# HSarham/automatic-ar

Hardware: AMD Instinct MI355X
Metric: LM iterations/sec (higher is better)
Workload: dtype f64

## Files before the change

automatic-ar_amd/csrc/ba_capi.hip:

```cpp
#include <hip/hip_runtime.h>
#include <dlfcn.h>
#include <execinfo.h>
#include <fcntl.h>
#include <unistd.h>
#include <signal.h>

#include <algorithm>
#include <array>
#include <atomic>
#include <chrono>
#include <cmath>
#include <cstring>
#include <map>
#include <numeric>
#include <condition_variable>
#include <mutex>
#include <vector>

#include "../host/internal.h"
#include "../host/se3.h"
#include "geom.hpp"
#include "hostcopy.h"
#include "kernels.h"

// ... 910 lines not shown
    return AAR_OK;
}

void aar_lm_default_params(aar_lm_params *p) {
    p->max_iters = 10000;
    p->min_error = 1e-5;
    p->min_step_error_diff = 0;
    p->min_average_step_error_diff = 1e-4;
    p->tau = 1;
    p->verbose = 0;
}

void aar_problem_destroy(aar_problem *pb) {
    if (!pb) return;
    (void)hipSetDevice(pb->device);
    if (pb->stream) (void)hipStreamSynchronize(pb->stream);
    for (void *p : pb->allocs) (void)hipFree(p);
    if (pb->h_scal) (void)hipHostFree(pb->h_scal);
    if (pb->h_pcg) (void)hipHostFree(pb->h_pcg);
    if (pb->h_gather) (void)hipHostFree(pb->h_gather);
    if (pb->up_ev) (void)hipEventDestroy(pb->up_ev);
    if (pb->ev[0]) (void)hipEventDestroy(pb->ev[0]);
    if (pb->ev[1]) (void)hipEventDestroy(pb->ev[1]);
    for (hipEvent_t e : pb->ev_pool) (void)hipEventDestroy(e);
    if (pb->ev_fork) (void)hipEventDestroy(pb->ev_fork);
    if (pb->ev_join) (void)hipEventDestroy(pb->ev_join);
    if (pb->stream2) { (void)hipStreamSynchronize(pb->stream2); (void)hipStreamDestroy(pb->stream2); }
    if (pb->stream) (void)hipStreamDestroy(pb->stream);
    delete pb;
}

void aar_solver_default_options(aar_solver_options *o) {
    if (!o) return;
    memset(o, 0, sizeof *o);
    o->struct_size = (uint32_t)sizeof *o;
    o->solver = AAR_SOLVER_AUTO;
}

int aar_problem_create(const aar_problem_desc *d, aar_problem **out) { return aar_problem_create_ex(d, nullptr, out); }

static int problem_create(const aar_problem_desc *d, const aar_solver_options *opts, const aar_problem_constraints *cons, aar_problem **out);
namespace {
aar_problem_constraints constraints_of(const aar_problem_constraints *c) {
    aar_problem_constraints k;
    memset(&k, 0, sizeof k);
    if (c) memcpy(&k, c, std::min<size_t>(c->struct_size, sizeof k));
    k.struct_size = (uint32_t)sizeof k;
    return k;
}
bool constraints_empty(const aar_problem_constraints &k) { return k.n_fixed_cams == 0 && k.n_fixed_markers == 0 && k.n_priors == 0; }
bool info_psd(const double *I) {
    double scale = 0;
    for (int i = 0; i < 36; i++) scale = std::max(scale, std::fabs(I[i]));
    for (int i = 0; i < 6; i++)
        for (int j = 0; j < i; j++)
            if (std::fabs(I[6 * i + j] - I[6 * j + i]) > 1e-12 * scale) return false;
    if (scale == 0) return true;
    const double tol = 1e-13 * scale;
    double Lm[36] = {0}, D[6];
    for (int k = 0; k < 6; k++) {
        double d = I[6 * k + k];
        for (int j = 0; j < k; j++) d -= Lm[6 * k + j] * Lm[6 * k + j] * D[j];
        if (d < -tol) return false;
        for (int i = k + 1; i < 6; i++) {
            double v = I[6 * i + k];
            for (int j = 0; j < k; j++) v -= Lm[6 * i + j] * Lm[6 * k + j] * D[j];
            if (d <= tol) {
                if (std::fabs(v) > std::sqrt(tol * scale)) return false;
                Lm[6 * i + k] = 0;
            } else {
                Lm[6 * i + k] = v / d;
            }
        }
        D[k] = d <= tol ? 0.0 : d;
    }
    return true;
}
}

int aar_problem_constraints_validate(const aar_problem_desc *d, const aar_problem_constraints *cons) {
    if (!d) return set_error(AAR_ERR_INVALID, "aar_problem_constraints_validate: null problem description");
    if (!cons) return AAR_OK;
    if (cons->struct_size < sizeof(uint32_t) + sizeof(int32_t)) return set_error(AAR_ERR_INVALID, "aar_problem_constraints.struct_size is not set");
    const aar_problem_constraints k = constraints_of(cons);
    const int C = d->num_cams, M = d->num_markers;
    if (k.n_fixed_cams < 0 || k.n_fixed_markers < 0 || k.n_priors < 0) return set_error(AAR_ERR_INVALID, "aar_problem_constraints: negative count");
    if ((k.n_fixed_cams && !k.fixed_cams) || (k.n_fixed_markers && !k.fixed_markers) || (k.n_priors && !k.priors))
        return set_error(AAR_ERR_INVALID, "aar_problem_constraints: null array with a non-zero count");
    std::vector<uint8_t> fixed((size_t)std::max(C, 0) + std::max(M, 0), 0);
    for (int c = 0; c < C; c++) fixed[c] = (c == d->root_cam || !d->optimize_cam_poses) ? 1 : 0;
    for (int m = 0; m < M; m++) fixed[(size_t)C + m] = (m == d->root_marker || !d->optimize_marker_poses) ? 1 : 0;
    for (int i = 0; i < k.n_fixed_cams; i++) {
        const int c = k.fixed_cams[i];
        if (c < 0 || c >= C) return set_error(AAR_ERR_INVALID, "fixed_cams[%d] = %d: camera index out of range [0, %d)", i, c, C);
        fixed[c] = 1;
    }
    for (int i = 0; i < k.n_fixed_markers; i++) {
        const int m = k.fixed_markers[i];
        if (m < 0 || m >= M) return set_error(AAR_ERR_INVALID, "fixed_markers[%d] = %d: marker index out of range [0, %d)", i, m, M);
        fixed[(size_t)C + m] = 1;
    }
    std::vector<int32_t> owner(fixed.size(), -1);
    for (int p = 0; p < k.n_priors; p++) {
        const aar_pose_prior &q = k.priors[p];
        const char *what = q.kind == AAR_PRIOR_CAMERA ? "camera" : "marker";
        if (q.kind != AAR_PRIOR_CAMERA && q.kind != AAR_PRIOR_MARKER) return set_error(AAR_ERR_INVALID, "priors[%d]: kind %d is not AAR_PRIOR_CAMERA or AAR_PRIOR_MARKER", p, q.kind);
        const int lim = q.kind == AAR_PRIOR_CAMERA ? C : M;
        if (q.index < 0 || q.index >= lim) return set_error(AAR_ERR_INVALID, "priors[%d]: %s index %d out of range [0, %d)", p, what, q.index, lim);
        const size_t e = q.kind == AAR_PRIOR_CAMERA ? (size_t)q.index : (size_t)C + q.index;
        if (owner[e] >= 0) return set_error(AAR_ERR_INVALID, "priors[%d]: %s index %d already has a prior (priors[%d])", p, what, q.index, owner[e]);
        owner[e] = p;
        if (fixed[e]) return set_error(AAR_ERR_INVALID, "priors[%d]: %s index %d is fixed (root, non-optimised group or fixed index)", p, what, q.index);
        for (int i = 0; i < 6; i++)
            if (!std::isfinite(q.x6[i])) return set_error(AAR_ERR_INVALID, "priors[%d]: x6[%d] is not finite", p, i);
        for (int i = 0; i < 36; i++)
            if (!std::isfinite(q.info[i])) return set_error(AAR_ERR_INVALID, "priors[%d]: info[%d] is not finite", p, i);
        if (!info_psd(q.info)) return set_error(AAR_ERR_INVALID, "priors[%d]: the information matrix is not symmetric positive semi-definite (its Cholesky fails)", p);
    }
    return AAR_OK;
}

int aar_problem_create_constrained(const aar_problem_desc *d, const aar_solver_options *opts, const aar_problem_constraints *cons, aar_problem **out) {
    if (!d || !out) return set_error(AAR_ERR_INVALID, "aar_problem_create_constrained: null argument");
    int rc = aar_problem_constraints_validate(d, cons);
    if (rc) return rc;
    if (!cons || constraints_empty(constraints_of(cons))) return aar_problem_create_ex(d, opts, out);
    const aar_problem_constraints k = constraints_of(cons);
    return problem_create(d, opts, &k, out);
}

int32_t aar_problem_num_priors(const aar_problem *pb) { return pb ? pb->P.n_prior : 0; }

static int abort_bt_fd = 2;
static void abort_backtrace(int sig) {
    void *bt[64];
    { char msg[64]; const int k = aar::g_last_kernel_id; int n = 0; const char *t = "last kernel id "; while (t[n]) { msg[n] = t[n]; n++; } if (k < 0) msg[n++] = '-'; else { if (k >= 10) msg[n++] = '0' + k / 10; msg[n++] = '0' + k % 10; } msg[n++] = '\n'; (void)!write(abort_bt_fd, msg, n); }
    const int n = backtrace(bt, 64);
    backtrace_symbols_fd(bt, n, abort_bt_fd);
    signal(sig, SIG_DFL);
    raise(sig);
}

int aar_problem_create_ex(const aar_problem_desc *d, const aar_solver_options *opts, aar_problem **out) { return problem_create(d, opts, nullptr, out); }

static int problem_create(const aar_problem_desc *d, const aar_solver_options *opts, const aar_problem_constraints *cons, aar_problem **out) {
    { static bool once = false; if (!once && getenv("AAR_ABORT_BACKTRACE")) { once = true; const int fd = open(getenv("AAR_ABORT_BACKTRACE"), O_WRONLY | O_CREAT | O_APPEND, 0644); if (fd >= 0) abort_bt_fd = fd; signal(SIGABRT, abort_backtrace); } }
    if (!d || !out) return set_error(AAR_ERR_INVALID, "aar_problem_create: null argument");
    aar_solver_options so;
    aar_solver_default_options(&so);
    if (opts) {
        if (opts->struct_size < 2 * sizeof(uint32_t)) return set_error(AAR_ERR_INVALID, "aar_solver_options.struct_size is not set (use aar_solver_default_options)");
        memcpy(&so, opts, std::min<size_t>(opts->struct_size, sizeof so));
        so.struct_size = (uint32_t)sizeof so;
    }
    int env_over = 0;
    if (const char *e = getenv("AAR_SOLVER")) {
        if (so.solver == AAR_SOLVER_AUTO) {
            int v = -1;
            if (!strcmp(e, "direct")) v = AAR_SOLVER_DIRECT;
            else if (!strcmp(e, "pcg")) v = AAR_SOLVER_PCG;
            else if (!strcmp(e, "spcg")) v = AAR_SOLVER_SPCG;
            if (v >= 0) { so.solver = v; env_over |= AAR_ENV_SOLVER; }
        }
    }
    if (const char *e = getenv("AAR_DETERMINISTIC")) if (!so.deterministic && atoi(e) != 0) { so.deterministic = 1; env_over |= AAR_ENV_DETERMINISTIC; }
    if (const char *e = getenv("AAR_PCG_ETA")) if (so.pcg_eta == 0 && atof(e) > 0) { so.pcg_eta = atof(e); env_over |= AAR_ENV_PCG_ETA; }
    if (const char *e = getenv("AAR_PCG_MAX_IT")) if (so.pcg_max_it == 0 && atoi(e) > 0) { so.pcg_max_it = atoi(e); env_over |= AAR_ENV_PCG_MAX_IT; }
    if (so.solver < AAR_SOLVER_DIRECT || so.solver > AAR_SOLVER_AUTO) return set_error(AAR_ERR_INVALID, "aar_solver_options.solver %d is not one of AAR_SOLVER_*", so.solver);
    if (so.pcg_eta < 0 || so.pcg_max_it < 0 || so.pcg_eta_loose < 0 || so.pcg_eta_switch < 0 || so.pcg_abs_tol < 0) return set_error(AAR_ERR_INVALID, "aar_solver_options: negative pcg_eta / pcg_eta_loose / pcg_eta_switch / pcg_abs_tol / pcg_max_it");
    const int C = d->num_cams, M = d->num_markers, Fg = d->num_frames;
    const int64_t Ng = d->num_obs;
    if (C < 1 || M < 1 || Fg < 0 || Ng < 0) return set_error(AAR_ERR_INVALID, "aar_problem_create: bad sizes");
    if (d->root_cam < 0 || d->root_cam >= C || d->root_marker < 0 || d->root_marker >= M)
        return set_error(AAR_ERR_INVALID, "aar_problem_create: root index out of range");
    if (!d->cam_mats || (Ng > 0 && (!d->obs_frame || !d->obs_cam || !d->obs_marker || !d->obs_uv)))
        return set_error(AAR_ERR_INVALID, "aar_problem_create: null array");
    if (Ng >= (1LL << 31) || (int64_t)C + M >= 32768) return set_error(AAR_ERR_UNSUPPORTED, "problem too large for 32-bit indexing");
    std::vector<int64_t> per_frame(Fg, 0);
    int64_t global_slots = 0;
    {
        std::vector<int32_t> seen_c(C, -1), seen_m(M, -1);
        for (int64_t o = 0; o < Ng; o++) {
            const int f = d->obs_frame[o], c = d->obs_cam[o], m = d->obs_marker[o];
            if (f < 0 || f >= Fg || c < 0 || c >= C || m < 0 || m >= M) return set_error(AAR_ERR_INVALID, "observation %lld has an index out of range", (long long)o);
            if (o > 0 && f < d->obs_frame[o - 1]) return set_error(AAR_ERR_INVALID, "observations must be ordered by frame (reference residual order)");
            per_frame[f]++;
            if (seen_c[c] != f) { seen_c[c] = f; global_slots += d->optimize_cam_intrinsics ? 2 : 1; }
            if (seen_m[m] != f) { seen_m[m] = f; global_slots += 1; }
        }
    }
    int rc = ensure_device(d->device_id);
    if (rc) return rc;

    aar_problem *pb = new aar_problem();
    pb->device = d->device_id;
    pb->comm = d->comm;
    aar_lm_default_params(&pb->prm);
    memset(&pb->times, 0, sizeof pb->times);
    const char *tenv = getenv("AAR_STAGE_TIMERS");
    pb->stage_timers = tenv && tenv[0] == '1';
    auto fail = [&](int code) { aar_problem_destroy(pb); return code; };
    if (hipStreamCreateWithFlags(&pb->stream, hipStreamNonBlocking) != hipSuccess) return fail(set_error(AAR_ERR_HIP, "hipStreamCreate failed"));
    (void)hipEventCreate(&pb->ev[0]);
    (void)hipEventCreate(&pb->ev[1]);
    if (hipStreamCreateWithFlags(&pb->stream2, hipStreamNonBlocking) != hipSuccess ||
        hipEventCreateWithFlags(&pb->ev_fork, hipEventDisableTiming) != hipSuccess ||
        hipEventCreateWithFlags(&pb->ev_join, hipEventDisableTiming) != hipSuccess)
        return fail(set_error(AAR_ERR_HIP, "second stream / events could not be created"));
    { const char *e = getenv("AAR_OVERLAP"); pb->overlap = (e && e[0] == '1'); }
    { const char *e = getenv("AAR_MERGE_PASSES"); if (e) pb->merge_passes = (e[0] != '0'); }
    { const char *e = getenv("AAR_FUSED_COMM"); if (e) pb->fused_comm = (e[0] != '0'); }
    { const char *e = getenv("AAR_SPEC_CHOL"); if (e) pb->spec_chol = (e[0] != '0'); }

    PoseLayout &L = pb->L;
    L.C = C; L.M = M; L.F = Fg; L.rc = d->root_cam; L.rm = d->root_marker;
    L.oc = d->optimize_cam_poses != 0; L.om = d->optimize_marker_poses != 0; L.of = d->optimize_object_poses != 0;
    L.oi = d->optimize_cam_intrinsics != 0;
    pb->N_global = Ng;

    const int world = pb->comm ? pb->comm->world : 1, rank = pb->comm ? pb->comm->rank : 0;
    pb->P.pcg_rank0 = rank == 0 ? 1 : 0;
    std::vector<int32_t> begin(world + 1, 0);
    if ((rc = aar_plan_shards(Fg, per_frame.data(), world, begin.data()))) return fail(rc);
    pb->f_begin = begin[rank];
    pb->f_end = begin[rank + 1];
    int64_t ob = 0;
    for (int f = 0; f < pb->f_begin; f++) ob += per_frame[f];
    int64_t N = 0;
    for (int f = pb->f_begin; f < pb->f_end; f++) N += per_frame[f];
    pb->o_begin = ob;

    DeviceProblem &P = pb->P;
    P.intr = L.oi ? 1 : 0;
    P.C = C; P.M = M; P.A = C + M + (L.oi ? C : 0); P.F = pb->f_end - pb->f_begin; P.N = N;
    P.n = 6 * P.A;
    P.nT = (P.n + CHOL_NB - 1) / CHOL_NB;
    P.n_pad = P.nT * CHOL_NB;
    P.spcg_root_c = (L.oc && C > 1) ? L.rc : -1;
    P.spcg_root_m = (L.om && M > 1) ? C + L.rm : -1;
    P.spcg_n_free = (L.oc ? C - 1 : 0) + (L.om ? M - 1 : 0) + (L.oi ? C : 0);
    P.res_f32 = d->residual_mode == AAR_RES_F64 ? 0 : 1;
    pb->with_huber = d->with_huber != 0;
    P.huber = pb->with_huber ? pb->hubber_delta : -1.f;
    P.half_size = (double)((float)d->marker_size / 2.f);
    P.frames_fixed = L.of ? 0 : 1;
    const int A = P.A, F = P.F;
    std::vector<int32_t> held(C + M, 0);
    bool held_extra = false;
    if (cons) {
        for (int i = 0; i < cons->n_fixed_cams; i++) { const int c = cons->fixed_cams[i]; if (c != L.rc && L.oc) { held[c] = 1; held_extra = true; } }
        for (int i = 0; i < cons->n_fixed_markers; i++) { const int m = cons->fixed_markers[i]; if (m != L.rm && L.om) { held[C + m] = 1; held_extra = true; } }
    }

    int local_rc = AAR_OK;
    std::vector<int32_t> frame_obs_start(F + 1, 0), fslot_start(F + 1, 0), fslot_ent;
    std::vector<ObsIdx> a_idx(N);
    std::vector<float> a_uv((size_t)8 * N);
    if (N) memcpy(a_uv.data(), d->obs_uv + 8 * ob, sizeof(float) * 8 * N);
    {
        int64_t o = 0;
        std::vector<int32_t> slot_of(A, -1);
        for (int f = 0; f < F; f++) {
            frame_obs_start[f] = (int32_t)o;
            const int64_t cnt = per_frame[pb->f_begin + f];
            std::vector<int32_t> ents;
            for (int64_t k = 0; k < cnt; k++) {
                const int64_t g = ob + o + k;
                ents.push_back(d->obs_cam[g]);
                ents.push_back(C + d->obs_marker[g]);
                if (L.oi) ents.push_back(C + M + d->obs_cam[g]);
            }
            std::sort(ents.begin(), ents.end());
            ents.erase(std::unique(ents.begin(), ents.end()), ents.end());
            if (ents.size() >= (1u << SLOT_C_BITS) && !local_rc) local_rc = set_error(AAR_ERR_UNSUPPORTED, "frame %d touches %zu entities (limit %d)", f, ents.size(), (1 << SLOT_C_BITS) - 1);
            for (size_t s = 0; s < ents.size(); s++) slot_of[ents[s]] = (int32_t)s;
            for (int64_t k = 0; k < cnt; k++) {
                const int64_t g = ob + o + k;
                ObsIdx id;
                id.frame = f; id.cam = d->obs_cam[g]; id.marker = C + d->obs_marker[g];
                id.slots = pack_slots(slot_of[id.cam], slot_of[id.marker], L.oi ? slot_of[C + M + id.cam] : 0);
                a_idx[o + k] = id;
            }
            fslot_start[f] = (int32_t)fslot_ent.size();
            fslot_ent.insert(fslot_ent.end(), ents.begin(), ents.end());
            P.max_kf = std::max<int>(P.max_kf, (int)ents.size());
            o += cnt;
        }
        frame_obs_start[F] = (int32_t)o;
        fslot_start[F] = (int32_t)fslot_ent.size();
    }
    P.total_slots = (int)fslot_ent.size();
    std::vector<int32_t> frame_stride(F, 1);
    for (int f = 0; f < F; f++) {
        const int n = frame_obs_start[f + 1] - frame_obs_start[f];
        if (n <= 16) continue;
        int st = n / 8 + 1;
        while (std::gcd(st, n) != 1) st++;
        frame_stride[f] = st;
    }
    {
        auto env_int = [](const char *name, int &v) { if (const char *e = getenv(name)) v = atoi(e); };
        env_int("AAR_FUSED_PANEL", P.tune.fused_panel); env_int("AAR_BS_RIDES", P.tune.bs_rides); env_int("AAR_BACKSUB_RIDES", P.tune.backsub_rides);
        env_int("AAR_LDL_LOOKAHEAD", P.tune.lookahead); env_int("AAR_PASSA_VARIANT", P.tune.passA_variant); env_int("AAR_PACK_SYSTEM", P.tune.pack_system);
        env_int("AAR_INIT_HEADSTART", P.tune.init_headstart); env_int("AAR_PASSB_LEAN", P.tune.passB_lean); env_int("AAR_PASSA_WRENCH", P.tune.passA_wrench); env_int("AAR_PASSB_WRENCH_MERGED", P.tune.passB_wrench_merged); env_int("AAR_SPCG_BACKSUB_RIDES", P.tune.spcg_backsub_rides); env_int("AAR_PASSAB_OCC2", P.tune.passAB_occ2);
    }
    const size_t ldsA = P.tune.passA_wrench ? passA_wrench_lds_bytes(P.max_kf, L.oi)
                                            : std::max(passA_lds_bytes(P.max_kf, 256), passA_lds_bytes(P.max_kf, 64));
    if (ldsA > 160 * 1024 && !local_rc) local_rc = set_error(AAR_ERR_UNSUPPORTED, "a frame touches %d cameras+markers: %zu bytes of LDS in the frame-block kernel (%s form), the CU has 160 KiB", P.max_kf, ldsA, P.tune.passA_wrench ? "wrench" : "row");
    P.deterministic = so.deterministic ? 1 : 0;
    { const char *e = getenv("AAR_DENSE_FROM_PASSA"); if (e) P.dense_from_passA = atoi(e) != 0 ? 1 : 0; }
    {
        hipDeviceProp_t prop;
        const int cus = (hipGetDeviceProperties(&prop, pb->device) == hipSuccess && prop.multiProcessorCount > 0) ? prop.multiProcessorCount : 64;
        P.n_cus = cus;
        const bool pcg_ok = pcg_lds_bytes(A) <= 150 * 1024;
        if (const char *t = getenv("AAR_SPCG_COARSE")) P.spcg_coarse = atoi(t) != 0;
        if (const char *t = getenv("AAR_SPCG_COARSE_FROM")) P.spcg_coarse_from = atoi(t);
        if (const char *t = getenv("AAR_PCG_COARSE")) P.pcg_coarse = atoi(t) != 0;
        if (const char *t = getenv("AAR_PCG_COARSE_FROM")) P.pcg_coarse_from = atoi(t);
        if (held_extra) { P.spcg_coarse = 0; P.pcg_coarse = 0; }
        P.pcg_e_every = P.total_slots >= 300000 ? 3 : 1;
        if (const char *t = getenv("AAR_PCG_E_EVERY")) P.pcg_e_every = std::max(1, atoi(t));
        if (const char *t = getenv("AAR_PCG_RESIDENT")) P.pcg_resident = atoi(t) != 0;
        if (pcg_lds_bytes(A, true) > 150 * 1024) P.pcg_coarse = 0;
        const int spcg_per_cu = spcg_fits(P.nT) ? spcg_resident_per_cu(P.nT, spcg_coarse_now(P)) : 0;
        const bool spcg_ok = spcg_fits(P.nT) && P.n_pad / 6 <= std::max(1, spcg_per_cu) * cus;
        int solver = so.solver;
        if (solver == AAR_SOLVER_AUTO) {
            const double kf_avg = Fg > 0 ? (double)global_slots / (double)Fg : 0.0;
            const bool pcg_pays = A >= 96 && pcg_ok && (double)global_slots / (double)world * (kf_avg - 30.0) >= 4e6;
            if (P.nT < 2) solver = AAR_SOLVER_DIRECT;
            else if (spcg_ok && !pcg_pays) solver = AAR_SOLVER_SPCG;
            else if (pcg_ok) solver = AAR_SOLVER_PCG;
            else solver = AAR_SOLVER_DIRECT;
        }
        pb->solver = solver;
        pb->env_overrides = env_over;
        P.use_pcg = solver == AAR_SOLVER_PCG ? 1 : 0;
        P.use_spcg = solver == AAR_SOLVER_SPCG ? 1 : 0;
        if (const char *t = getenv("AAR_SPCG_SPREAD")) P.spcg_spread = std::max(1, atoi(t));
        if (P.n_pad / 6 > std::min(4, std::max(1, spcg_per_cu)) * (cus / 8)) P.spcg_spread = 1;
        P.pcg_eta = P.use_spcg ? SPCG_ETA_DEFAULT : PCG_ETA_DEFAULT;
        if (so.pcg_eta > 0) P.pcg_eta = so.pcg_eta;
        P.pcg_eta_loose = 0.0;
        if (so.pcg_eta_loose > 0) P.pcg_eta_loose = so.pcg_eta_loose;
        else if (so.pcg_eta == 0 && (P.use_pcg || P.use_spcg)) P.pcg_eta_loose = P.use_pcg ? PCG_ETA_LOOSE_DEFAULT : SPCG_ETA_LOOSE_DEFAULT;
        if (const char *e = getenv("AAR_PCG_ETA_LOOSE")) if (so.pcg_eta_loose == 0) P.pcg_eta_loose = atof(e);
        if (P.pcg_eta_loose <= P.pcg_eta) P.pcg_eta_loose = 0.0;
        P.pcg_abs_tol = P.use_pcg ? PCG_ABS_TOL_DEFAULT : SPCG_ABS_TOL_DEFAULT;
        if (so.pcg_abs_tol > 0) P.pcg_abs_tol = so.pcg_abs_tol;
        else if (const char *e = getenv("AAR_PCG_ABS_TOL")) P.pcg_abs_tol = atof(e);
        if (so.pcg_eta_switch > 0) P.pcg_eta_switch = so.pcg_eta_switch;
        else if (const char *e = getenv("AAR_PCG_ETA_SWITCH")) P.pcg_eta_switch = atof(e);
        P.pcg_eta_now = P.pcg_eta;
        P.spcg_max_it = spcg_default_cap(P.nT);
        if (so.pcg_max_it > 0) { P.pcg_max_it = so.pcg_max_it; P.spcg_max_it = std::min(so.pcg_max_it, SPCG_MAX_IT); }
        if (P.use_pcg && !pcg_ok && !local_rc) local_rc = set_error(AAR_ERR_UNSUPPORTED, "AAR_SOLVER_PCG keeps the CG vectors and the preconditioner of %d unknowns in LDS: too many shared entities", 6 * A);
        if (P.use_spcg && !spcg_ok && !local_rc) local_rc = set_error(AAR_ERR_UNSUPPORTED, "AAR_SOLVER_SPCG keeps the reduced system in the registers of one wavefront per shared entity: %d unknowns are too many (limit %d, and at most %d entities)", 6 * A, 96 * SPCG_MAX_NT, std::max(1, spcg_per_cu) * cus);
    }
    bool schur_mfma = A >= 96 && F > 0;
    if (const char *e = getenv("AAR_SCHUR_MFMA")) schur_mfma = atoi(e) != 0 && F > 0;
    if (P.deterministic) schur_mfma = false;
    if (P.use_pcg) schur_mfma = true;
    if (schur_mfma) {
        const size_t panel_bytes = (size_t)2 * F * ((A + 1 + 31) / 32 * 32) * 288;
        size_t free_b = 0, total_b = 0;
        size_t budget = (hipMemGetInfo(&free_b, &total_b) == hipSuccess) ? free_b / 2 : (size_t)64 << 30;
        if (const char *e = getenv("AAR_SCHUR_PANEL_MB")) budget = (size_t)std::max(0, atoi(e)) << 20;
        if (panel_bytes > budget) schur_mfma = false;
    }
    if (!schur_mfma && (size_t)A * 36 * 8 + 2048 > 160 * 1024 && !local_rc)
        local_rc = set_error(AAR_ERR_UNSUPPORTED, "%d cameras+markers exceed the row panel the output-stationary Schur kernel holds in LDS (and the dense panels of the MFMA kernel do not fit the memory budget)", A);
    {
        if (pb->comm && (rc = dev_alloc(pb, &pb->d_status, 1))) return fail(rc);
        int agreed = local_rc;
        if ((rc = collective_status(pb, local_rc, &agreed))) return fail(rc);
        if (local_rc) return fail(local_rc);
        if (agreed) return fail(set_error(agreed, "another rank could not create its shard of the problem (status %d)", agreed));
    }

    std::vector<int32_t> perm(N);
    std::iota(perm.begin(), perm.end(), 0);
    std::stable_sort(perm.begin(), perm.end(), [&](int32_t x, int32_t y) {
        const ObsIdx &p = a_idx[x], &q = a_idx[y];
        if (p.cam != q.cam) return p.cam < q.cam;
        if (p.marker != q.marker) return p.marker < q.marker;
        return p.frame < q.frame;
    });
    std::vector<ObsIdx> b_idx(N);
    std::vector<float> b_uv((size_t)8 * N);
    for (int64_t i = 0; i < N; i++) {
        b_idx[i] = a_idx[perm[i]];
        memcpy(&b_uv[8 * i], &a_uv[8 * (size_t)perm[i]], 8 * sizeof(float));
    }
    int chunk_len = (int)((N / 2048 + 63) / 64 * 64);
    chunk_len = std::min(std::max(chunk_len, 64), 512);
    if (const char *e = getenv("AAR_PASSB_CHUNK")) chunk_len = std::min(std::max(atoi(e) / 64 * 64, 64), PASSB_CHUNK);
    std::vector<int32_t> chunk_start;
    for (int64_t i = 0; i < N;) {
        int64_t e = i;
        while (e < N && b_idx[e].cam == b_idx[i].cam && b_idx[e].marker == b_idx[i].marker) e++;
        for (int64_t s = i; s < e; s += chunk_len) chunk_start.push_back((int32_t)s);
        i = e;
    }
    P.n_chunks = (int)chunk_start.size();
    chunk_start.push_back((int32_t)N);

    std::vector<int32_t> up_start(A + 1, 0), up_ent;
    {
        std::vector<std::vector<int32_t>> nb(A);
        for (int ch = 0; ch < P.n_chunks; ch++) {
            const ObsIdx &h = b_idx[chunk_start[ch]];
            if (ch > 0 && b_idx[chunk_start[ch - 1]].cam == h.cam && b_idx[chunk_start[ch - 1]].marker == h.marker) continue;
            int ents[3] = {h.cam, h.marker, L.oi ? C + M + h.cam : -1};
            for (int x = 0; x < 3; x++)
                for (int y = 0; y < 3; y++)
                    if (x != y && ents[x] >= 0 && ents[y] >= 0) nb[ents[x]].push_back(ents[y]);
        }
        for (int a = 0; a < A; a++) {
            std::sort(nb[a].begin(), nb[a].end());
            nb[a].erase(std::unique(nb[a].begin(), nb[a].end()), nb[a].end());
            up_start[a] = (int32_t)up_ent.size();
            up_ent.insert(up_ent.end(), nb[a].begin(), nb[a].end());
        }
        up_start[A] = (int32_t)up_ent.size();
        if (up_ent.empty()) up_ent.push_back(0);
    }

    std::vector<std::vector<std::pair<int32_t, int32_t>>> inc(A);
    for (int f = 0; f < F; f++)
        for (int s = fslot_start[f]; s < fslot_start[f + 1]; s++) inc[fslot_ent[s]].push_back({f, s});
    std::vector<int4> pair_rec;
    std::vector<int32_t> sw_ent, sw_begin, sw_end;
    const int64_t total_pairs = P.total_slots;
    int per_item = (int)std::min<int64_t>(64, std::max<int64_t>(16, total_pairs / 1024));
    per_item = (per_item + 3) / 4 * 4;
    if (const char *e = getenv("AAR_SCHUR_ITEM")) per_item = std::max(4, atoi(e));
    std::vector<int> pair_base(A + 1, 0);
    for (int a = 0; a < A; a++) {
        pair_base[a] = (int)pair_rec.size();
        for (auto &pr : inc[a]) pair_rec.push_back(make_int4(pr.first, pr.second, fslot_start[pr.first], 0));
    }
    pair_base[A] = (int)pair_rec.size();
    int window = 0;
    if (total_pairs >= 262144) window = 64;
    if (const char *e = getenv("AAR_SCHUR_WINDOW")) window = std::max(0, atoi(e));
    if (window > 0) {
        std::vector<int> cursor(A, 0);
        for (int f0 = 0; f0 < F; f0 += window)
            for (int a = 0; a < A; a++) {
                int c = cursor[a];
                const int cnt = (int)inc[a].size();
                int e = c;
                while (e < cnt && inc[a][e].first < f0 + window) e++;
                if (e > c) {
                    sw_ent.push_back(a);
                    sw_begin.push_back(pair_base[a] + c);
                    sw_end.push_back(pair_base[a] + e);
                }
                cursor[a] = e;
            }
    } else {
        int xcd = 1;
        if (const char *e = getenv("AAR_SCHUR_XCD")) xcd = atoi(e) != 0 ? 8 : 1;
        std::vector<std::vector<std::array<int32_t, 3>>> lists(xcd);
        for (int a = 0; a < A; a++) {
            const int cnt = (int)inc[a].size();
            int s = 0;
            for (int x = 0; x < xcd; x++) {
                const int f_hi = (int)((int64_t)F * (x + 1) / xcd);
                int e = s;
                while (e < cnt && inc[a][e].first < f_hi) e++;
                for (int c = s; c < e; c += per_item)
                    lists[x].push_back({(int32_t)a, (int32_t)(pair_base[a] + c), (int32_t)(pair_base[a] + std::min(e, c + per_item))});
                s = e;
            }
        }
        size_t longest = 0;
        for (auto &l : lists) longest = std::max(longest, l.size());
        for (size_t k = 0; k < longest; k++)
            for (int x = 0; x < xcd; x++) {
                if (k < lists[x].size()) { sw_ent.push_back(lists[x][k][0]); sw_begin.push_back(lists[x][k][1]); sw_end.push_back(lists[x][k][2]); }
                else if (xcd > 1) { sw_ent.push_back(0); sw_begin.push_back(0); sw_end.push_back(0); }
            }
    }
    P.n_swork = (int)sw_ent.size();
    std::vector<int64_t> sp_off;
    std::vector<int32_t> se_start, se_items, pbr_start, pbr_chunk, pbr_kind, pbr_a, pbr_b;
    int64_t sp_total = 0;
    if (P.deterministic) {
        sp_off.resize(sw_ent.size());
        std::vector<std::vector<int32_t>> items(A);
        for (size_t w = 0; w < sw_ent.size(); w++) {
            sp_off[w] = sp_total;
            sp_total += ((int64_t)(sw_ent[w] + 1) * 36 + 8);
            items[sw_ent[w]].push_back((int32_t)w);
        }
        se_start.assign(A + 1, 0);
        for (int a = 0; a < A; a++) {
            std::sort(items[a].begin(), items[a].end(), [&](int32_t x, int32_t y) { return sw_begin[x] < sw_begin[y]; });
            se_start[a] = (int32_t)se_items.size();
            se_items.insert(se_items.end(), items[a].begin(), items[a].end());
        }
        se_start[A] = (int32_t)se_items.size();
        std::vector<std::vector<int32_t>> by_cam(C), by_mk(A);
        pbr_start.push_back(0);
        auto emit = [&](int kind, int ea, int eb, const std::vector<int32_t> &chs) {
            if (chs.empty()) return;
            pbr_chunk.insert(pbr_chunk.end(), chs.begin(), chs.end());
            pbr_start.push_back((int32_t)pbr_chunk.size());
            pbr_kind.push_back(kind); pbr_a.push_back(ea); pbr_b.push_back(eb);
        };
        std::vector<int32_t> run;
        for (int ch = 0; ch < P.n_chunks; ch++) {
            const ObsIdx &h = b_idx[chunk_start[ch]];
            by_cam[h.cam].push_back(ch);
            by_mk[h.marker].push_back(ch);
            run.push_back(ch);
            const bool last = ch + 1 == P.n_chunks || b_idx[chunk_start[ch + 1]].cam != h.cam || b_idx[chunk_start[ch + 1]].marker != h.marker;
            if (last) { emit(2, h.cam, h.marker, run); run.clear(); }
        }
        for (int c = 0; c < C; c++) emit(0, c, 0, by_cam[c]);
        for (int m = 0; m < A; m++) emit(1, m, 0, by_mk[m]);
        P.n_pbr = (int)pbr_kind.size();
        P.pb_stride = L.oi ? 152 : 90;
    }
    std::vector<int32_t> sm_ga, sm_gb, sm_fb, sm_fe, slot_frame, slot_dense, dense_ent;
    std::vector<int32_t> sm_frames;
    if (schur_mfma && !P.use_pcg) {
        std::vector<int32_t> seen;
        for (int a = 0; a < A; a++)
            if (!inc[a].empty()) seen.push_back(a);
        std::stable_sort(seen.begin(), seen.end(), [&](int32_t x, int32_t y) { return inc[x].size() > inc[y].size(); });
        std::vector<int32_t> dense_of(A, -1);
        dense_ent.push_back(-1);
        for (int32_t a : seen) { dense_of[a] = (int32_t)dense_ent.size(); dense_ent.push_back(a); }
        P.Ad = ((int)dense_ent.size() + 31) / 32 * 32;
        dense_ent.resize(P.Ad, -1);
        const int nga = P.Ad / 16, ngb = P.Ad / 32;
        std::vector<std::vector<uint8_t>> pa(nga, std::vector<uint8_t>(F, 0)), pb(ngb, std::vector<uint8_t>(F, 0));
        for (int f = 0; f < F; f++) {
            pa[0][f] = pb[0][f] = 1;
            for (int s = fslot_start[f]; s < fslot_start[f + 1]; s++) {
                const int dd = dense_of[fslot_ent[s]];
                pa[dd / 16][f] = 1;
                pb[dd / 32][f] = 1;
            }
        }
        struct Blk { int ga, gb; std::vector<int32_t> fr; };
        std::vector<Blk> blks;
        int64_t total_steps = 0;
        for (int ga = 0; ga < nga; ga++)
            for (int gb = 0; gb <= (16 * ga + 15) / 32; gb++) {
                Blk bk{ga, gb, {}};
                for (int f = 0; f < F; f++)
                    if (pa[ga][f] && pb[gb][f]) bk.fr.push_back(f);
                if (bk.fr.empty()) continue;
                total_steps += ((int64_t)bk.fr.size() + 1) / 2;
                blks.push_back(std::move(bk));
            }
        int target = 12 * (int)blks.size();
        if (const char *e = getenv("AAR_SCHUR_SPLIT")) target = std::max(1, atoi(e)) * (int)blks.size();
        const int64_t plen = std::max<int64_t>(16, ((2 * total_steps + target - 1) / target + 3) / 4 * 4);
        struct Piece { int blk; int64_t b, e; int f0; };
        std::vector<Piece> pieces;
        for (size_t k = 0; k < blks.size(); k++)
            for (int64_t b0 = 0; b0 < (int64_t)blks[k].fr.size(); b0 += plen)
                pieces.push_back({(int)k, b0, std::min<int64_t>(b0 + plen, (int64_t)blks[k].fr.size()), blks[k].fr[b0]});
        std::stable_sort(pieces.begin(), pieces.end(), [](const Piece &x, const Piece &y) { return x.f0 < y.f0; });
        for (const Piece &pc : pieces) {
            sm_ga.push_back(blks[pc.blk].ga); sm_gb.push_back(blks[pc.blk].gb);
            sm_fb.push_back((int32_t)sm_frames.size());
            sm_frames.insert(sm_frames.end(), blks[pc.blk].fr.begin() + pc.b, blks[pc.blk].fr.begin() + pc.e);
            sm_fe.push_back((int32_t)sm_frames.size());
        }
        slot_frame.resize(P.total_slots);
        slot_dense.resize(P.total_slots);
        for (int f = 0; f < F; f++)
            for (int s = fslot_start[f]; s < fslot_start[f + 1]; s++) {
                slot_frame[s] = f;
                slot_dense[s] = dense_of[fslot_ent[s]];
            }
        P.n_smwork = (int)sm_ga.size();
    }

    std::vector<int32_t> ent_fixed(A, 0);
    for (int c = 0; c < C; c++) ent_fixed[c] = (c == L.rc || !L.oc) ? 1 : 0;
    for (int m = 0; m < M; m++) ent_fixed[C + m] = (m == L.rm || !L.om) ? 1 : 0;
    for (int e = 0; e < C + M; e++) ent_fixed[e] |= held[e];
    std::vector<double> Kh(d->cam_mats, d->cam_mats + 9 * (size_t)C);

#define UP(field, vec) if ((rc = dev_upload(pb, &P.field, vec))) return fail(rc)
    UP(K, Kh); UP(a_idx, a_idx); UP(a_uv, a_uv); UP(frame_obs_start, frame_obs_start); UP(frame_stride, frame_stride);
    UP(fslot_start, fslot_start); UP(fslot_ent, fslot_ent); UP(b_idx, b_idx); UP(b_uv, b_uv);
    UP(chunk_start, chunk_start); UP(ent_fixed, ent_fixed); UP(up_start, up_start); UP(up_ent, up_ent);
    UP(sw_ent, sw_ent); UP(sw_begin, sw_begin); UP(sw_end, sw_end); UP(pair_rec, pair_rec);
    if (P.use_pcg) {
        const int cus = P.n_cus;
        int64_t longest = 0;
        for (int a = 0; a < A; a++) longest = std::max<int64_t>(longest, pair_base[a + 1] - pair_base[a]);
        int64_t chunk = std::max<int64_t>(256, (total_pairs + 2LL * cus - 1) / (2LL * cus));
        chunk = std::max<int64_t>(chunk, (longest + 7) / 8);
        if (const char *t = getenv("AAR_PCG_CHUNK")) chunk = std::max<int64_t>((longest + 7) / 8, atoll(t));
        std::vector<int32_t> it_ent, it_begin, it_end, ent_item_start(A + 1, 0);
        for (int a = 0; a < A; a++) {
            ent_item_start[a] = (int32_t)it_ent.size();
            const int64_t b0 = pair_base[a], e0 = ent_fixed[a] ? pair_base[a] : pair_base[a + 1];
            int64_t b = b0;
            do {
                const int64_t e = std::min<int64_t>(e0, b + chunk);
                it_ent.push_back(a); it_begin.push_back((int32_t)b); it_end.push_back((int32_t)e);
                b = e;
            } while (b < e0);
        }
        ent_item_start[A] = (int32_t)it_ent.size();
        P.pcg_n_items = (int)it_ent.size();
        UP(pcg_it_ent, it_ent); UP(pcg_it_begin, it_begin); UP(pcg_it_end, it_end); UP(pcg_ent_item_start, ent_item_start);
    }
    if (P.deterministic) { UP(sp_off, sp_off); UP(se_start, se_start); UP(se_items, se_items); UP(pbr_start, pbr_start); UP(pbr_chunk, pbr_chunk); UP(pbr_kind, pbr_kind); UP(pbr_a, pbr_a); UP(pbr_b, pbr_b); }
    if (P.n_smwork) { UP(sm_ga, sm_ga); UP(sm_gb, sm_gb); UP(sm_fb, sm_fb); UP(sm_fe, sm_fe); UP(slot_dense, slot_dense); UP(slot_frame, slot_frame); UP(dense_ent, dense_ent); UP(sm_frames, sm_frames); }
#undef UP
#define AL(field, count) if ((rc = dev_alloc(pb, &P.field, (size_t)(count)))) return fail(rc)
    AL(z[0], 6 * (size_t)(A + F)); AL(z[1], 6 * (size_t)(A + F));
    AL(ent[0], (size_t)(A + F) * ENT_STRIDE); AL(ent[1], (size_t)(A + F) * ENT_STRIDE);
    for (int w = 0; w < 2; w++) {
        AL(blk[w].V, (size_t)F * 36); AL(blk[w].gf, (size_t)F * 6); AL(blk[w].W, (size_t)P.total_slots * 36);
        AL(blk[w].Vinv, (size_t)F * 36); AL(blk[w].hf, (size_t)F * 6);
        AL(blk[w].S, (size_t)P.n_pad * P.n_pad + 2 * (size_t)P.n_pad + 8);
        P.blk[w].rhs = P.blk[w].S + (size_t)P.n_pad * P.n_pad;
        P.blk[w].g0 = P.blk[w].rhs + P.n_pad;
        P.blk[w].tail = P.blk[w].g0 + P.n_pad;
        if (hipMemset(P.blk[w].tail, 0, 8 * sizeof(double)) != hipSuccess) return fail(set_error(AAR_ERR_HIP, "hipMemset failed"));
    }
    if (P.deterministic) { AL(sp_part, (size_t)sp_total); AL(pb_part, (size_t)P.n_chunks * P.pb_stride); }
    if (P.use_pcg) {
        AL(pcg_ws, (size_t)P.pcg_n_items * 28 + 6 * (size_t)F + 8); AL(pcg_counter, 8);
        AL(pcg_yg, (size_t)3 * PCG_NYV * P.n_pad + (size_t)28 * A + 160 + 8); AL(pcg_hop, 2 * PCG_HOP_WORDS);
        if (const char *t = getenv("AAR_PCG_FUSED")) P.pcg_fused = atoi(t) != 0 ? 1 : 0;
        {
            int w32 = 1;
            if (const char *t = getenv("AAR_PCG_W32")) w32 = atoi(t) != 0 ? 1 : 0;
            if (w32 && P.pcg_fused && !P.deterministic && P.pcg_eta >= PCG_W32_MIN_ETA)
                for (int w = 0; w < 2; w++) AL(blk[w].Wf, (size_t)P.total_slots * 36 + 4);
        }
        P.pcg_grid = P.n_cus;
        const int64_t want = std::max<int64_t>(32, ((int64_t)F + 3) / 4);
        P.pcg_grid = (int)std::min<int64_t>(P.pcg_grid, want);
        if (pb->comm) {
            AL(pcgd_setup, (size_t)A * 28 + 152); AL(pcgd_minv, (size_t)A * 36 + 72 + (size_t)12 * A + 8);
            AL(pcgd_state, 2 * (18 * (size_t)A + 8)); AL(pcgd_y, 3 * (6 * (size_t)A + 8));
            if (hipHostMalloc((void **)&pb->h_pcg, 8 * sizeof(double), hipHostMallocMapped | hipHostMallocCoherent) != hipSuccess)
                return fail(set_error(AAR_ERR_HIP, "hipHostMalloc failed"));
            memset(pb->h_pcg, 0, 8 * sizeof(double));
            if (hipHostGetDevicePointer((void **)&P.pcgd_host, pb->h_pcg, 0) != hipSuccess) return fail(set_error(AAR_ERR_HIP, "hipHostGetDevicePointer failed"));
        }
        if (const char *t = getenv("AAR_PCG_GRID")) P.pcg_grid = std::max(1, atoi(t));
        P.pcg_grid = std::min(P.pcg_grid, pcg_max_grid(A, P.pcg_coarse != 0, P.n_cus));
    }
    if (P.use_spcg) {
        AL(spcg_ws, spcg_ws_doubles(P.n_pad)); AL(spcg_iters, 8); AL(spcg_done, 2);
        if (spcg_coarse_now(P)) AL(spcg_pre, spcg_pre_doubles(P.n_pad));
        spcg_ws_reset(P, pb->stream);
    }
    if (P.n_smwork) { AL(Wd, (size_t)F * P.Ad * 36); AL(Yd, (size_t)F * P.Ad * 36); }
    AL(Dfac, (size_t)P.nT * CHOL_NB * CHOL_NB); AL(Linv16, (size_t)P.nT * (CHOL_NB / 16) * 256); AL(delta_s, P.n_pad); AL(bs_flags, (size_t)P.nT + 1);
    AL(Lp, (size_t)P.nT * P.n_pad * CHOL_NB); AL(zf, P.n_pad);
    AL(err_part, std::max<size_t>((size_t)F, (size_t)((N + 255) / 256)) + 1);
    AL(lin_part, 2 * (size_t)(F + 1)); AL(scal, 8); AL(flags, 4);
    if (cons && cons->n_priors > 0) {
        const int np_ = cons->n_priors;
        std::vector<int32_t> pent(np_);
        std::vector<double> pdat((size_t)np_ * PRIOR_DAT);
        for (int p = 0; p < np_; p++) {
            const aar_pose_prior &q = cons->priors[p];
            pent[p] = q.kind == AAR_PRIOR_CAMERA ? q.index : C + q.index;
            memcpy(&pdat[(size_t)p * PRIOR_DAT], q.x6, 6 * sizeof(double));
            memcpy(&pdat[(size_t)p * PRIOR_DAT + 6], q.info, 36 * sizeof(double));
        }
        if ((rc = dev_upload(pb, &P.prior_ent, pent)) || (rc = dev_upload(pb, &P.prior_dat, pdat))) return fail(rc);
        AL(prior_out, (size_t)np_ * 8 + 1);
        P.n_prior = np_;
        P.prior_rank0 = rank == 0 ? 1 : 0;
        pb->priors.assign(cons->priors, cons->priors + np_);
    }
#undef AL
    if ((rc = dev_alloc(pb, &pb->d_diag, P.n_pad))) return fail(rc);
    if (pb->comm && (rc = dev_alloc(pb, &pb->d_frames_all, 6 * (size_t)std::max(Fg, 1)))) return fail(rc);
    if (pb->comm && (rc = dev_alloc(pb, &pb->d_pack, (size_t)P.n_pad * (P.n_pad + 1) / 2 + 2 * (size_t)P.n_pad + 8))) return fail(rc);
    if (hipHostMalloc((void **)&pb->h_scal, 16 * sizeof(double), hipHostMallocMapped | hipHostMallocCoherent) != hipSuccess)
        return fail(set_error(AAR_ERR_HIP, "hipHostMalloc failed"));
    memset(pb->h_scal, 0, 16 * sizeof(double));
    if (hipHostGetDevicePointer((void **)&P.host_result, pb->h_scal, 0) != hipSuccess)
        return fail(set_error(AAR_ERR_HIP, "hipHostGetDevicePointer failed"));
    if (hipStreamSynchronize(pb->stream) != hipSuccess) return fail(set_error(AAR_ERR_HIP, "upload failed"));
    {
        if (pb->h_z.reserve((size_t)6 * (A + F))) return fail(set_error(AAR_ERR_HIP, "hipHostMalloc(pose staging) failed"));
        if (hipEventCreateWithFlags(&pb->up_ev, hipEventDisableTiming) != hipSuccess) { pb->up_ev = nullptr; (void)hipGetLastError(); }
        if (hipMemcpyAsync(pb->h_z.data(), P.z[0], (size_t)6 * (A + F) * sizeof(double), hipMemcpyDeviceToHost, pb->stream) != hipSuccess ||
            hipStreamSynchronize(pb->stream) != hipSuccess)
            return fail(set_error(AAR_ERR_HIP, "device-to-host copy failed"));
    }
    pb->h_fslot_start = fslot_start;
    pb->h_fslot_ent = fslot_ent;
    pb->h_ent_fixed = ent_fixed;
    *out = pb;
    return AAR_OK;
}

int64_t aar_problem_full_len(const aar_problem *pb) { return pb->L.full_len(); }
int64_t aar_problem_num_vars(const aar_problem *pb) { return pb->L.z_len(); }
int64_t aar_problem_local_obs(const aar_problem *pb) { return pb->P.N; }

int aar_problem_set_huber_delta(aar_problem *pb, float delta) {
    if (!pb || !(delta > 0.f)) return set_error(AAR_ERR_INVALID, "aar_problem_set_huber_delta: bad argument");
    pb->hubber_delta = delta;
    if (pb->with_huber) pb->P.huber = delta;
    return AAR_OK;
}
float aar_problem_get_huber_delta(const aar_problem *pb) { return pb ? pb->hubber_delta : 0.f; }

int aar_eval_residuals(aar_problem *pb, const double *x_full, double *r, double *sum_sq) {
    if (!pb || !x_full) return set_error(AAR_ERR_INVALID, "aar_eval_residuals: null argument");
    if (r && pb->comm) return set_error(AAR_ERR_UNSUPPORTED, "residual vector output is single-GPU only");
    HIP_TRY(hipSetDevice(pb->device));
    DeviceProblem &P = pb->P;
    int rc = upload_z(pb, x_full, pb->cur);
    if (rc) return rc;
    double *d_r = nullptr;
    if (r) HIP_TRY(hipMalloc((void **)&d_r, std::max<size_t>(1, 8 * (size_t)P.N) * sizeof(double)));
    launch_unpack(P, pb->cur, pb->stream);
    launch_residual(P, pb->cur, d_r, pb->stream);
    HIP_TRY(hipMemsetAsync(P.lin_part, 0, 2 * (size_t)(P.F + 1) * sizeof(double), pb->stream));
    launch_reduce_scalars(P, residual_blocks(P), false, 0ull, pb->stream);
    rc = allreduce(pb, P.scal, 1, NCCL_SUM);
    if (rc) { if (d_r) (void)hipFree(d_r); return rc; }
    pb->seq++;
    launch_publish(P, pb->seq, pb->stream);
    HIP_TRY(hipStreamSynchronize(pb->stream));
    if (r && (rc = copy_d2h(pb, r, d_r, 8 * (size_t)P.N * sizeof(double)))) { (void)hipFree(d_r); return rc; }
    if ((rc = wait_result(pb))) { if (d_r) (void)hipFree(d_r); return rc; }
    if (d_r) (void)hipFree(d_r);
    if (sum_sq) *sum_sq = pb->h_scal[0];
    pb->lm_ready = false;
    return check_async("residual kernels");
}

int aar_reproj_stats(aar_problem *pb, const double *x_full, double *rmse, double *sum_sq) {
    if (!pb) return set_error(AAR_ERR_INVALID, "aar_reproj_stats: null argument");
    const int saved = pb->P.res_f32;
    const float saved_h = pb->P.huber;
    pb->P.res_f32 = 0;
    pb->P.huber = -1.f;
    double ss = 0;
    int rc = aar_eval_residuals(pb, x_full, nullptr, &ss);
    pb->P.res_f32 = saved;
    pb->P.huber = saved_h;
    if (rc) return rc;
    if (sum_sq) *sum_sq = ss;
    if (rmse) *rmse = std::sqrt(ss / (4.0 * (double)pb->N_global));
    return AAR_OK;
}

int aar_eval_normal_equations(aar_problem *pb, const double *x_full, double *JtJ, double *B, double *sum_sq) {
    if (!pb || !x_full) return set_error(AAR_ERR_INVALID, "aar_eval_normal_equations: null argument");
    if (pb->comm) return set_error(AAR_ERR_UNSUPPORTED, "dense normal-equation output is single-GPU only");
    HIP_TRY(hipSetDevice(pb->device));
    DeviceProblem &P = pb->P;
    const PoseLayout &L = pb->L;
    int rc = upload_z(pb, x_full, pb->cur);
    if (rc) return rc;
    if ((rc = zero_block_set(pb, pb->cur))) return rc;
    P.want_w64 = 1;
    rc = eval_blocks(pb, pb->cur, -1.0, -1);
    P.want_w64 = 0;
    if (rc) return rc;
    const int A = P.A, F = P.F, np = P.n_pad;
    const DeviceProblem::Blocks &bk = P.blk[pb->cur];
    std::vector<double> U0((size_t)np * np), g0(np), V((size_t)F * 36), gf((size_t)F * 6), W((size_t)P.total_slots * 36), ep(n_err_terms(P));
    HIP_TRY(hipStreamSynchronize(pb->stream));
    if ((rc = copy_d2h(pb, U0.data(), bk.S, U0.size() * sizeof(double))) || (rc = copy_d2h(pb, g0.data(), bk.g0, g0.size() * sizeof(double)))) return rc;
    if (F) {
        if ((rc = copy_d2h(pb, V.data(), bk.V, V.size() * sizeof(double))) || (rc = copy_d2h(pb, gf.data(), bk.gf, gf.size() * sizeof(double))) ||
            (rc = copy_d2h(pb, W.data(), bk.W, W.size() * sizeof(double)))) return rc;
    }
    if (!ep.empty() && (rc = copy_d2h(pb, ep.data(), P.err_part, ep.size() * sizeof(double)))) return rc;
    pb->lm_ready = false;
    const int64_t Pz = L.z_len();
    auto par_col = [&](int a, int i) -> int64_t {
        if (a < L.C) { const int s = L.cam_slot(a); return (s < 0 || !L.oc) ? -1 : L.z_cam0() + 6LL * s + i; }
        if (a < L.C + L.M) { const int s = L.mk_slot(a - L.C); return (s < 0 || !L.om) ? -1 : L.z_mk0() + 6LL * s + i; }
        return i < 4 ? L.z_intr0() + 9LL * (a - L.C - L.M) + i : -1;
    };
    if (JtJ) {
        std::fill(JtJ, JtJ + Pz * Pz, 0.0);
        for (int a = 0; a < A; a++)
            for (int b = 0; b <= a; b++)
                for (int i = 0; i < 6; i++)
                    for (int j = 0; j < 6; j++) {
                        if (a == b && j > i) continue;
                        const int64_t ca = par_col(a, i), cb = par_col(b, j);
                        if (ca < 0 || cb < 0) continue;
                        const double v = U0[(size_t)(6 * a + i) * np + 6 * b + j];
                        JtJ[ca * Pz + cb] = v;
                        JtJ[cb * Pz + ca] = v;
                    }
        if (L.of)
            for (int f = 0; f < F; f++) {
                const int64_t cf = L.z_fr0() + 6LL * f;
                for (int i = 0; i < 6; i++)
                    for (int j = 0; j < 6; j++) JtJ[(cf + i) * Pz + cf + j] = V[(size_t)f * 36 + i * 6 + j];
                for (int s = pb->h_fslot_start[f]; s < pb->h_fslot_start[f + 1]; s++)
                    for (int i = 0; i < 6; i++) {
                        const int64_t ca = par_col(pb->h_fslot_ent[s], i);
                        if (ca < 0) continue;
                        for (int j = 0; j < 6; j++) {
                            const double v = W[(size_t)s * 36 + i * 6 + j];
                            JtJ[ca * Pz + cf + j] = v;
                            JtJ[(cf + j) * Pz + ca] = v;
                        }
                    }
            }
    }
    if (B) {
        std::fill(B, B + Pz, 0.0);
        for (int a = 0; a < A; a++)
            for (int i = 0; i < 6; i++) {
                const int64_t ca = par_col(a, i);
                if (ca >= 0) B[ca] = g0[6 * (size_t)a + i];
            }
        if (L.of)
            for (int f = 0; f < F; f++)
                for (int i = 0; i < 6; i++) B[L.z_fr0() + 6LL * f + i] = gf[(size_t)f * 6 + i];
    }
    if (sum_sq) {
        double s = 0;
        for (double v : ep) s += v;
        *sum_sq = s;
    }
    return AAR_OK;
}

int aar_problem_eval_priors(aar_problem *pb, const double *x_full, double *e_out, double *cost) {
    if (!pb || !x_full) return set_error(AAR_ERR_INVALID, "aar_problem_eval_priors: null argument");
    HIP_TRY(hipSetDevice(pb->device));
    DeviceProblem &P = pb->P;
    if (P.n_prior == 0) {
        if (cost) *cost = 0.0;
        return AAR_OK;
    }
    int rc = upload_z(pb, x_full, pb->cur);
    if (rc) return rc;
    pb->lm_ready = false;
    pb->blocks_valid = false;
    launch_unpack(P, pb->cur, pb->stream);
    launch_prior(P, pb->cur, false, pb->stream);
    pb->launches += 2;
    if ((rc = check_async("prior kernels"))) return rc;
    HIP_TRY(hipStreamSynchronize(pb->stream));
    std::vector<double> h((size_t)P.n_prior * 8 + 1);
    if ((rc = copy_d2h(pb, h.data(), P.prior_out, h.size() * sizeof(double)))) return rc;
    if (e_out)
        for (int p = 0; p < P.n_prior; p++) memcpy(e_out + 6 * (size_t)p, &h[8 * (size_t)p], 6 * sizeof(double));
    if (cost) *cost = h[(size_t)P.n_prior * 8];
    return AAR_OK;
}

int aar_eval_damped_step(aar_problem *pb, const double *x_full, double mu, double *delta) {
    if (!pb || !x_full || !delta) return set_error(AAR_ERR_INVALID, "aar_eval_damped_step: null argument");
    HIP_TRY(hipSetDevice(pb->device));
    const PoseLayout &L = pb->L;
    int rc = upload_z(pb, x_full, pb->cur);
    if (rc) return rc;
    if ((rc = zero_block_set(pb, pb->cur))) return rc;
    if ((rc = eval_blocks(pb, pb->cur, -1.0, -1))) return rc;
    pb->vinv_mu = -1;
    pb->schur_mu = -1;
    pb->s_reduced = pb->trial_reduced = false;
    pb->spcg_skip = pb->spcg_backoff = 0;
    pb->last_cg_its = -1;
    pb->near_cap_tries = 0;
    pb->P.spcg_coarse_on = 0;
    pb->P.pcg_e_age = 0;
    if (pb->P.use_pcg && pb->P.pcg_counter) HIP_TRY(hipMemsetAsync(pb->P.pcg_counter + 2, 0, sizeof(int32_t), pb->stream));
    pb->P.pcg_eta_now = pb->P.pcg_eta;
    if ((rc = damped_try_fb(pb, mu, false))) return rc == TRY_NOT_POSITIVE_DEFINITE ? AAR_ERR_NUMERIC : rc;
    pb->lm_ready = false;
    std::vector<double> x0(x_full, x_full + L.full_len()), x1(x0);
    if ((rc = download_z(pb, 1 - pb->cur, x1.data()))) return rc;
    std::vector<double> z0((size_t)std::max<int64_t>(L.z_len(), 1)), z1(z0);
    extract_z(L, x0.data(), z0.data());
    extract_z(L, x1.data(), z1.data());
    for (int64_t i = 0; i < L.z_len(); i++) delta[i] = z1[i] - z0[i];
    return AAR_OK;
}

int aar_problem_covariance(aar_problem *pb, const double *x_full, double *entity_cov, double *entity_diag, double *frame_cov,
                           aar_covariance_report *report) {
    if (!pb || !x_full) return set_error(AAR_ERR_INVALID, "aar_problem_covariance: null argument");
    if (report && report->struct_size < sizeof(uint32_t)) return set_error(AAR_ERR_INVALID, "aar_problem_covariance: report->struct_size not set");
    HIP_TRY(hipSetDevice(pb->device));
    DeviceProblem &P = pb->P;
    const PoseLayout &L = pb->L;
    const int cur = pb->cur, np = P.n_pad, n2 = P.n_pad + CHOL_NB, nT2 = P.nT + 1, NB = CHOL_NB;
    int rc = upload_z(pb, x_full, cur);
    if (rc) return rc;
    if ((rc = zero_block_set(pb, cur))) return rc;
    pb->lm_ready = false;
    pb->blocks_valid = false;
    pb->vinv_mu = pb->schur_mu = -1;
    pb->s_reduced = pb->trial_reduced = false;
    pb->spec_chol_blk = -1;
    if (pb->panels_blk == cur) pb->panels_blk = -1;
    P.want_w64 = 1;
    rc = eval_blocks(pb, cur, -1.0, -1);
    P.want_w64 = 0;
    if (rc) return rc;
    launch_frame_inv(P, cur, 0.0, pb->stream);
    launch_schur(P, cur, 1.0, pb->stream, 0, 0, nullptr, false);
    launch_reduce_scalars(P, n_err_terms(P), false, 0ull, pb->stream, P.blk[cur].tail);
    pb->launches += 3;
    if (pb->comm && (rc = allreduce_system(pb, cur, 1))) return rc;
    const size_t fr = (size_t)std::max(P.F, 1) * 36;
    const size_t o_S2 = 0, o_D = o_S2 + (size_t)n2 * n2 + 2 * (size_t)n2 + 8, o_Li = o_D + (size_t)nT2 * NB * NB, o_Lp = o_Li + (size_t)nT2 * (NB / 16) * 256,
                 o_zf = o_Lp + (size_t)nT2 * n2 * NB, o_ds = o_zf + n2, o_Lc = o_ds + n2, o_X = o_Lc + (size_t)np * np, o_Si = o_X + (size_t)np * np,
                 o_Dv = o_Si + (size_t)np * np, o_fr = o_Dv + np, o_db = o_fr + fr, total = o_db + 36 * (size_t)std::max(P.A, 1);
    if (!pb->cov_ws) {
        if ((rc = dev_alloc(pb, &pb->cov_ws, total))) return rc;
        if ((rc = dev_alloc(pb, &pb->cov_iws, (size_t)np + nT2 + 1 + 4))) return rc;
    }
    double *ws = pb->cov_ws;
    int32_t *rowmask = pb->cov_iws, *bsf = rowmask + np, *flg = bsf + nT2 + 1;
    HIP_TRY(hipMemcpy2DAsync(pb->d_diag, sizeof(double), P.blk[cur].S, (size_t)(np + 1) * sizeof(double), sizeof(double), np, hipMemcpyDeviceToDevice, pb->stream));
    std::vector<double> diag(np);
    double sum_sq = 0;
    HIP_TRY(hipStreamSynchronize(pb->stream));
    if ((rc = copy_d2h(pb, diag.data(), pb->d_diag, np * sizeof(double))) || (rc = copy_d2h(pb, &sum_sq, P.blk[cur].tail, sizeof(double)))) return rc;
    auto par_col = [&](int a, int i) -> int64_t {
        if (a < L.C) { const int s = L.cam_slot(a); return (s < 0 || !L.oc) ? -1 : L.z_cam0() + 6LL * s + i; }
        if (a < L.C + L.M) { const int s = L.mk_slot(a - L.C); return (s < 0 || !L.om) ? -1 : L.z_mk0() + 6LL * s + i; }
        return i < 4 ? L.z_intr0() + 9LL * (a - L.C - L.M) + i : -1;
    };
    std::vector<int32_t> mask(np, 1);
    for (int a = 0; a < P.A; a++) {
        bool seen = false;
        for (int i = 0; i < 6; i++) seen |= par_col(a, i) >= 0 && diag[6 * a + i] != 0.0;
        const bool held = a < L.C + L.M && pb->h_ent_fixed[a];
        for (int i = 0; i < 6; i++) mask[6 * a + i] = (seen && !held && par_col(a, i) >= 0) ? 0 : 1;
    }
    if ((rc = copy_h2d(pb, rowmask, mask.data(), np * sizeof(int32_t)))) return rc;
    double *S2 = ws + o_S2;
    launch_cov_stage(P.blk[cur].S, np, S2, n2, rowmask, pb->stream);
    HIP_TRY(hipMemsetAsync(S2 + (size_t)n2 * n2, 0, (2 * (size_t)n2 + 8) * sizeof(double), pb->stream));
    HIP_TRY(hipMemsetAsync(bsf, 0, (nT2 + 1 + 4) * sizeof(int32_t), pb->stream));
    DeviceProblem Q = P;
    Q.n_pad = n2; Q.nT = nT2;
    Q.blk[cur].S = S2; Q.blk[cur].rhs = S2 + (size_t)n2 * n2; Q.blk[cur].g0 = Q.blk[cur].rhs + n2; Q.blk[cur].tail = Q.blk[cur].g0 + n2;
    Q.Dfac = ws + o_D; Q.Linv16 = ws + o_Li; Q.Lp = ws + o_Lp; Q.zf = ws + o_zf; Q.delta_s = ws + o_ds; Q.bs_flags = bsf; Q.bs_epoch = 0; Q.flags = flg;
    (void)launch_chol(Q, cur, 0.0, pb->stream, -1);
    launch_cov_inverse(S2, Q.Dfac, Q.Lp, np, n2, nT2, P.tune.fused_panel, ws + o_Lc, ws + o_Dv, ws + o_X, ws + o_Si, pb->stream);
    const bool frames = frame_cov && L.of && P.F > 0;
    if (frames) launch_cov_frames(P, cur, ws + o_Si, rowmask, ws + o_fr, pb->stream);
    if (entity_diag && !entity_cov) launch_cov_diag_blocks(ws + o_Si, np, P.A, ws + o_db, pb->stream);
    pb->launches += 4 + 3 * nT2 + np / 32;
    if ((rc = check_async("covariance kernels"))) return rc;
// ... 1274 lines not shown
```

automatic-ar_amd/csrc/kernels.h:

```cpp
#pragma once
#include <hip/hip_runtime.h>
#include <stdint.h>
#include <utility>

namespace aar {

constexpr int CHOL_NB = 96;
constexpr int PASSB_CHUNK = 1024;
constexpr int SPCG_MAX_IT = 128, SPCG_BUFS = SPCG_MAX_IT + 2, SPCG_MAX_NT = 14;
inline int spcg_default_cap(int nT) { return nT <= 4 ? 64 : SPCG_MAX_IT; }
constexpr int PCG_NY = 16;
constexpr int PCG_NYV = 2;
constexpr int PCG_HOP_WORDS = (2 * PCG_NY + 1) * 16;
constexpr double PCG_W32_MIN_ETA = 1e-4;
constexpr double SPCG_ABS_TOL_DEFAULT = 2e-5, PCG_ABS_TOL_DEFAULT = 5e-5;
constexpr double SPCG_ETA_DEFAULT = 3e-4, SPCG_ETA_LOOSE_DEFAULT = 0.0, PCG_ETA_DEFAULT = 5e-3, PCG_ETA_LOOSE_DEFAULT = 0.0;
inline int spcg_stride(int n_pad) { return 8 * (n_pad / 6); }


#ifndef SPCG_PRE
#define SPCG_PRE 0
#endif

enum KernelId { KID_UNPACK = 0, KID_RESIDUAL, KID_PASSA, KID_PASSB, KID_MAXDIAG, KID_FRAME_INV, KID_SCHUR, KID_LDL_DIAG,
                KID_LDL_TRSM, KID_LDL_UPDATE, KID_LDL_BACKSOLVE, KID_BACKSUB, KID_REDUCE, KID_LDL_PANEL, KID_PCG, KID_SPCG, KID_SPCG_PRE, KID_PRIOR, KID_COUNT };

struct LaunchHook {
    void (*pre)(void *ctx, int kid) = nullptr;
    void (*post)(void *ctx, int kid) = nullptr;
    void *ctx = nullptr;
};

struct ObsIdx {
    int32_t frame, cam, marker, slots;
};

struct DeviceProblem {
    int C = 0, M = 0, A = 0;
    int intr = 0;
    int F = 0;
    int64_t N = 0;
    int n = 0, n_pad = 0, nT = 0;
    int total_slots = 0, max_kf = 0;
    int n_chunks = 0, n_swork = 0;
    int res_f32 = 1;
    float huber = -1.f;
    double half_size = 0;
    double *K = nullptr;
    ObsIdx *a_idx = nullptr;
    float *a_uv = nullptr;
    int32_t *frame_obs_start = nullptr;
    int32_t *frame_stride = nullptr;
    int32_t *fslot_start = nullptr;
    int32_t *fslot_ent = nullptr;
    ObsIdx *b_idx = nullptr;
    float *b_uv = nullptr;
    int32_t *chunk_start = nullptr;
    int32_t *ent_fixed = nullptr;
    int frames_fixed = 0;
    int32_t *sw_ent = nullptr, *sw_begin = nullptr, *sw_end = nullptr;
    int4 *pair_rec = nullptr;
    int n_smwork = 0;
    int32_t *sm_ga = nullptr, *sm_gb = nullptr, *sm_fb = nullptr, *sm_fe = nullptr, *sm_frames = nullptr;
    int Ad = 0;
    int32_t *slot_dense = nullptr;
    int32_t *slot_frame = nullptr;
    int32_t *dense_ent = nullptr;
    double *Wd = nullptr, *Yd = nullptr;
    int dense_from_passA = 1;
    int deterministic = 0;
    double *pb_part = nullptr;
    int pb_stride = 0, n_pbr = 0;
    int32_t *pbr_start = nullptr, *pbr_chunk = nullptr, *pbr_kind = nullptr, *pbr_a = nullptr, *pbr_b = nullptr;
    double *sp_part = nullptr;
    int64_t *sp_off = nullptr;
    int32_t *se_start = nullptr, *se_items = nullptr;
    int use_pcg = 0, pcg_grid = 0, pcg_max_it = 200;
    double pcg_eta = 0.1;
    double pcg_eta_loose = 0.0, pcg_eta_switch = 0.01, pcg_eta_now = 0.1;
    double pcg_abs_tol = SPCG_ABS_TOL_DEFAULT;
    int pcg_n_items = 0;
    int32_t *pcg_it_ent = nullptr, *pcg_it_begin = nullptr, *pcg_it_end = nullptr, *pcg_ent_item_start = nullptr;
    double *pcg_ws = nullptr;
    int32_t *pcg_counter = nullptr;
    mutable int pcg_parity = 0;
    int n_cus = 256;
    mutable int want_w64 = 0;
    int pcg_fused = 1;
    int pcg_rank0 = 1;
    int pcg_resident = 1;
    int pcg_e_every = 1;
    mutable int pcg_e_age = 0;
    int pcg_coarse = 1, pcg_coarse_from = 8;
    int32_t *up_start = nullptr, *up_ent = nullptr;
    double *pcg_yg = nullptr;
    int32_t *pcg_hop = nullptr;
    int use_spcg = 0, spcg_max_it = 64;
    int spcg_spread = 8;
    int spcg_coarse = 1;
    int spcg_coarse_from = 12;
    mutable int spcg_coarse_on = 0;
    double *spcg_pre = nullptr;
    mutable int spcg_pre_epoch = 0;
    int spcg_root_c = -1, spcg_root_m = -1, spcg_n_free = 0;
    int spcg_test_drop = -1;
    double *spcg_ws = nullptr;
    int32_t *spcg_iters = nullptr;
    mutable int spcg_parity = 0;
    int32_t *spcg_done = nullptr;
    mutable int spcg_epoch = 0;
    double *pcgd_setup = nullptr, *pcgd_minv = nullptr, *pcgd_state = nullptr, *pcgd_y = nullptr, *pcgd_host = nullptr;
    struct Tuning {
        int fused_panel = 3;
        int bs_rides = 1;
        int backsub_rides = 0;
        int lookahead = 1;
        int passA_variant = 0;
        int passAB_occ2 = -1;
        int spcg_backsub_rides = 0;
        int passA_wrench = 1;
        int passB_wrench_merged = 0;
        int passB_lean = 0;
        int pack_system = -1;
        int init_headstart = 1;
    } tune;
    double *z[2] = {nullptr, nullptr};
    double *ent[2] = {nullptr, nullptr};
    struct Blocks {
        double *V = nullptr, *gf = nullptr;
        double *W = nullptr;
        float *Wf = nullptr;
        double *Vinv = nullptr, *hf = nullptr;
        double *S = nullptr;
        double *rhs = nullptr;
        double *g0 = nullptr;
        double *tail = nullptr;
    } blk[2];
    double *Dfac = nullptr;
    double *Linv16 = nullptr;
    double *Lp = nullptr;
    double *zf = nullptr;
    double *delta_s = nullptr;
    int32_t *bs_flags = nullptr;
    mutable int bs_epoch = 0;
    double *err_part = nullptr;
    double *lin_part = nullptr;
    double *scal = nullptr;
    double *host_result = nullptr;
    int32_t *flags = nullptr;
    double *r_out = nullptr;
    int n_prior = 0, prior_rank0 = 1;
    int32_t *prior_ent = nullptr;
    double *prior_dat = nullptr;
    double *prior_out = nullptr;
    LaunchHook hook;
};

void raise_dynamic_lds(const void *kernel, size_t bytes);
template <typename... Params, typename... Args>
inline void launch_lds(void (*kernel)(Params...), dim3 grid, dim3 block, size_t lds, hipStream_t st, Args &&...args) {
    raise_dynamic_lds(reinterpret_cast<const void *>(kernel), lds);
    hipLaunchKernelGGL(kernel, grid, block, lds, st, std::forward<Args>(args)...);
}

struct KTable { const double *base; int stride; };
constexpr int ENT_STRIDE_H = 24;
inline KTable k_table(const DeviceProblem &P, int which) {
    if (P.intr) return KTable{P.ent[which] + (size_t)(P.C + P.M) * ENT_STRIDE_H, ENT_STRIDE_H};
    return KTable{P.K, 9};
}
constexpr int SLOT_C_BITS = 10, SLOT_M_BITS = 11;
inline int pack_slots(int sc, int sm, int sk) { return sc | (sm << SLOT_C_BITS) | (sk << (SLOT_C_BITS + SLOT_M_BITS)); }

extern volatile int g_last_kernel_id;
struct HookScope {
    const DeviceProblem &P;
    int kid;
    HookScope(const DeviceProblem &p, int k) : P(p), kid(k) { g_last_kernel_id = k; if (P.hook.pre) P.hook.pre(P.hook.ctx, kid); }
    ~HookScope() { if (P.hook.post) P.hook.post(P.hook.ctx, kid); }
};

void launch_unpack(const DeviceProblem &P, int which, hipStream_t st, int zero_blk = -1);
void launch_residual(const DeviceProblem &P, int which, double *r_out, hipStream_t st);
void launch_passA(const DeviceProblem &P, int which, double mu_pred, int zero_blk, hipStream_t st);
void launch_passB(const DeviceProblem &P, int which, hipStream_t st);
bool launch_passAB(const DeviceProblem &P, int which, double mu_pred, int zero_blk, hipStream_t st);
size_t passA_lds_bytes(int max_kf, int block);
size_t passA_wrench_lds_bytes(int max_kf, bool intr);
void launch_maxdiag(const DeviceProblem &P, int which, hipStream_t st);
void launch_frame_inv(const DeviceProblem &P, int which, double mu, hipStream_t st, const double *mu_dev = nullptr, double mu_scale = 0.0);
bool launch_schur(const DeviceProblem &P, int which, double sign, hipStream_t st, unsigned long long ride_seq = 0, int ride_n_err = 0,
                  double *ride_scal = nullptr, bool panels_ready = false);
bool launch_chol(const DeviceProblem &P, int which, double mu, hipStream_t st, int trial = -1);
void launch_backsub(const DeviceProblem &P, int cur, int trial, hipStream_t st);
void launch_pcg(const DeviceProblem &P, int which, double mu, hipStream_t st);
size_t pcg_lds_bytes(int A, bool coarse = false);
int pcg_max_grid(int A, bool coarse, int cus);
bool launch_spcg(const DeviceProblem &P, int which, double mu, hipStream_t st, int trial = -1);
int spcg_resident_per_cu(int nT, bool coarse);
inline bool spcg_coarse_now(const DeviceProblem &P) { return P.spcg_coarse && (P.spcg_root_c >= 0 || P.spcg_root_m >= 0); }
bool spcg_fits(int nT);
size_t spcg_ws_doubles(int n_pad);
size_t spcg_pre_doubles(int n_pad);
void spcg_ws_reset(const DeviceProblem &P, hipStream_t st);
void launch_pcgd_setup(const DeviceProblem &P, int which, double mu, hipStream_t st);
void launch_pcgd_iter(const DeviceProblem &P, int which, double mu, int k, bool last, unsigned long long publish_seq, hipStream_t st);
double *pcgd_y_of_launch(const DeviceProblem &P, int k);
void launch_reduce_scalars(const DeviceProblem &P, int n_err, bool fold_shared, unsigned long long publish_seq, hipStream_t st,
                           double *scal_out = nullptr, int maxdiag_blk = -1);
void launch_publish(const DeviceProblem &P, unsigned long long publish_seq, hipStream_t st, const double *src = nullptr, bool flags_reduced = false);
int residual_blocks(const DeviceProblem &P);
constexpr int PRIOR_DAT = 42;
void launch_prior(const DeviceProblem &P, int which, bool add, hipStream_t st);
inline int n_err_terms(const DeviceProblem &P) { return P.F + ((P.n_prior > 0 && P.prior_rank0) ? 1 : 0); }
void launch_track(const DeviceProblem &P, int which, int max_iters, double min_error, double min_step, double min_avg, double tau,
                  int32_t *iters_out, double *err_out, hipStream_t st);

constexpr int SMOOTH_TAIL = 256;
struct SmoothWork {
    double *z[2] = {nullptr, nullptr};
    double *delta = nullptr;
    double *Dg = nullptr, *Of = nullptr;
    double *rhs = nullptr;
    double *Dw = nullptr, *Uw = nullptr, *bw = nullptr, *Dinv = nullptr, *Ls = nullptr;
    double *Ef[2] = {nullptr, nullptr}, *Pe[2] = {nullptr, nullptr};
    double *lin = nullptr;
    double *lam = nullptr;
    double *rel_buf = nullptr;
    const double *rel = nullptr;
    double *res = nullptr;
    int32_t *flag = nullptr;
};
size_t smooth_work_doubles(int F);
void smooth_work_carve(SmoothWork &w, double *base, int F);
void launch_smooth_eval(const DeviceProblem &P, int which, const SmoothWork &w, int cur, bool with_j, hipStream_t st);
int launch_smooth_solve(const SmoothWork &w, int F, double mu, hipStream_t st);

constexpr int LIVE_MAX_W = 16;
constexpr int LIVE_HDR_BYTES = 64;
constexpr int LIVE_REC_BYTES = 48;
constexpr int LIVE_RES_DOUBLES = 24;
constexpr int LIVE_INFO_DOUBLES = 16;
inline size_t live_slot_bytes(int max_obs) {
    return (LIVE_HDR_BYTES + (size_t)(LIVE_REC_BYTES + sizeof(int32_t)) * (size_t)max_obs + 15) / 16 * 16;
}
struct LiveArgs {
    const double *ent, *Kmat;
    const char *ring;
    size_t slot_bytes;
    double *zslot;
    double *anchor;
    double *Ef, *Pe;
    double *res;
    float huber; double h;
    int max_iters; double min_error, min_step_error_diff, min_average_step_error_diff, tau;
    int W, slots, first_slot;
    int has_anchor, smooth, has_init;
    double rows;
    int cnt[LIVE_MAX_W];
    double lam[LIVE_MAX_W][2];
    int anchor_pair;
    int marginal, has_marginal;
    int covariance;
    double *unc;
};
constexpr int LIVE_UNC_VALID = 0, LIVE_UNC_HAS = 1, LIVE_UNC_DROP = 2, LIVE_UNC_LM = 4, LIVE_UNC_M = 40, LIVE_UNC_HDR = 48;
constexpr int LIVE_UNC_DOUBLES = LIVE_UNC_HDR + 36 * LIVE_MAX_W;
constexpr double LIVE_MARGINAL_PIVOT_REL = 1e-10;
void launch_live_push(const LiveArgs &a, hipStream_t st);

constexpr int LIVE_START_VOTE = 1, LIVE_START_BEST = 2;
struct LiveInitArgs {
    char *slot;
    int n_det;
    const void *cams;
    const double *Tcr, *Tmr;
    int C;
    float hf; double h;
    double threshold;
    int do_vote, policy, has_init, has_prev;
    const double *zprev;
    const double *ent, *Kmat; float huber; double h_track;
    double *poses; int *has2;
    double *Tc, *BJ, *cost; int *fin;
    double *info;
};
void launch_live_init(const LiveInitArgs &a, hipStream_t st);

void launch_cov_stage(const double *S, int n_pad, double *S2, int n2, const int32_t *rowmask, hipStream_t st);
void launch_cov_inverse(const double *S2, const double *Dfac, const double *Lp, int n_pad, int n2, int nT2, int fused_m, double *Lc, double *Dinv,
                        double *X, double *Sinv, hipStream_t st);
void launch_cov_diag_blocks(const double *Sinv, int n_pad, int A, double *out, hipStream_t st);
void launch_cov_frames(const DeviceProblem &P, int which, const double *Sinv, const int32_t *rowmask, double *out, hipStream_t st);

constexpr int RR_DIGIT_BITS = 11, RR_BINS = 1 << RR_DIGIT_BITS, RR_PASSES = 6;
struct RRSel {
    unsigned long long prefix, rank;
    double t;
    int pshift, done, single, pad;
};
struct RRWork {
    double *err = nullptr, *ss = nullptr, *fstat = nullptr, *rstat = nullptr, *esum = nullptr, *emax = nullptr, *hd = nullptr;
    uint8_t *keep = nullptr;
    int32_t *perm = nullptr, *run_start = nullptr, *cam_run_start = nullptr, *mk_run_start = nullptr, *mk_runs = nullptr;
    unsigned long long *rmax = nullptr;
    uint32_t *hist = nullptr;
    RRSel *sel = nullptr;
    int R = 0;
};
constexpr int RR_HIST_WORDS = RR_BINS + 3;
void launch_rr_errors(const DeviceProblem &P, int which, const RRWork &w, unsigned long long rank, hipStream_t st);
void launch_rr_select_pass(const DeviceProblem &P, const RRWork &w, hipStream_t st);
void launch_rr_to_double(const RRWork &w, hipStream_t st);
void launch_rr_pick(const RRWork &w, bool reduced, hipStream_t st);
void launch_rr_stats(const DeviceProblem &P, const RRWork &w, int has_rule, double k_median, double min_px, hipStream_t st);

__device__ __forceinline__ double encode_flags(int f) {
    return (double)(f & 1) + 4096.0 * (double)((f >> 1) & 1) + 16777216.0 * (double)((f >> 2) & 1) + 68719476736.0 * (double)((f >> 3) & 1);
}
__device__ __forceinline__ int decode_flags(double v) {
    const long long q = (long long)v;
    return ((q % 4096) ? 1 : 0) | (((q / 4096) % 4096) ? 2 : 0) | (((q / 16777216) % 4096) ? 4 : 0) | ((q / 68719476736LL) ? 8 : 0);
}

__device__ __forceinline__ void publish_host(const double *__restrict__ scal, const int32_t *__restrict__ flags,
                                             double *__restrict__ host, unsigned long long seq, int flags_reduced = 0) {
#pragma unroll
    for (int i = 0; i < 8; i++) host[i] = scal[i];
    reinterpret_cast<long long *>(host)[8] = flags_reduced ? (long long)decode_flags(scal[3]) : (long long)(flags[0] | flags[1] | flags[2] | flags[3]);
    __threadfence_system();
    __hip_atomic_store(reinterpret_cast<unsigned long long *>(host) + 9, seq, __ATOMIC_RELEASE, __HIP_MEMORY_SCOPE_SYSTEM);
}


}
```

automatic-ar_amd/csrc/spcg_kernels.hip:

```cpp
#include "geom.hpp"
#include "kernels.h"
#include "backsub.hpp"
#include "wave.hpp"

namespace aar {

namespace {

constexpr unsigned long long SPCG_EMPTY = 0xFFF85EEDFFF85EEDull;

__device__ __forceinline__ bool sp_empty(double v) { return (unsigned long long)__double_as_longlong(v) == SPCG_EMPTY; }
__device__ __forceinline__ void sp_st(double *p, double v) { __hip_atomic_store(p, v, __ATOMIC_RELAXED, __HIP_MEMORY_SCOPE_AGENT); }
__device__ __forceinline__ void sp_st_xcd(double *p, double v) { __hip_atomic_store(p, v, __ATOMIC_RELAXED, __HIP_MEMORY_SCOPE_WORKGROUP); }
__device__ __forceinline__ double sp_ld(const double *p) { return __hip_atomic_load(p, __ATOMIC_RELAXED, __HIP_MEMORY_SCOPE_AGENT); }

__device__ __forceinline__ double rl(double v, int l) {
    return __hiloint2double(__builtin_amdgcn_readlane(__double2hiint(v), l), __builtin_amdgcn_readlane(__double2loint(v), l));
}

}

#ifdef AAR_STAMPS
__device__ unsigned long long g_sp_stamps[512];
__device__ int g_sp_polls[80];
#define SP_STAMP(k) do { __builtin_amdgcn_sched_barrier(0); if (e == e0 && lane == 0 && (k) < 512) g_sp_stamps[k] = __builtin_amdgcn_s_memtime(); __builtin_amdgcn_sched_barrier(0); } while (0)
#define SP_VAL(k, v) do { if (e == e0 && lane == 0 && (k) < 512) g_sp_stamps[k] = (unsigned long long)__double_as_longlong(v); } while (0)
#else
#define SP_STAMP(k) do { } while (0)
#define SP_VAL(k, v) do { } while (0)
#endif

struct SpcgArgs {
    const double *S, *rhs, *g0;
    const int32_t *ent_fixed;
    int n, n_pad;
    double mu, eta2;
    double abs2_mu;
    int max_it;
    double *ws;
    long long set_len;
    int stride, parity;
    double *x_out;
    int32_t *iters;
    int32_t *flags;
    int spread;
    int ride, n_ent_total, n_riders;
    BacksubArgs bs;
    int32_t *done;
    int done_epoch;
    int test_drop;
    const double *pre_rows, *pre_minv, *pre_z, *pre_azt, *pre_share;
    int root_c, root_m;
    int C, M;
};

typedef unsigned int sp_u32x4 __attribute__((ext_vector_type(4)));

template <int NT, bool CO>
__global__ void __launch_bounds__(64) k_spcg(const SpcgArgs a) {
    constexpr int NPAD = 96 * NT, NK = 6 * NT, NENT = 16 * NT, NL = NT, NEB = (NENT + 63) / 64;
    __shared__ __align__(16) double mv[NPAD];
    if (blockIdx.x % a.spread || (int)blockIdx.x >= a.n_ent_total * a.spread) {
        if (!a.ride || blockIdx.x % 8 == 0) return;
        __shared__ double red[32];
        const int bx = (int)blockIdx.x, cg_range = a.n_ent_total * a.spread;
        const int rid = bx < cg_range ? bx - bx / a.spread - 1 : a.n_ent_total * (a.spread - 1) + (bx - cg_range) - (bx - cg_range + 7) / 8;
        for (int blk = rid; blk <= a.bs.n_frame_blocks; blk += a.n_riders) backsub_body(a.bs, blk, red, a.done + 1, a.done_epoch, a.flags);
        return;
    }
    const int lane = threadIdx.x, e = blockIdx.x / a.spread, i = lane >> 3, g = lane & 7;
    auto leave = [&]() {
        if (!a.ride) return;
        asm volatile("s_waitcnt vmcnt(0)" ::: "memory");
        if (lane == 0) {
            const int old = __hip_atomic_fetch_add(a.done, 1, __ATOMIC_RELAXED, __HIP_MEMORY_SCOPE_AGENT);
            if (old + 1 == a.done_epoch * a.n_ent_total) __hip_atomic_store(a.done + 1, a.done_epoch, __ATOMIC_RELAXED, __HIP_MEMORY_SCOPE_AGENT);
        }
    };
    const int n_free_ent = a.n / 6;
    auto fixed = [&](int ent) -> bool { return ent >= n_free_ent || (a.ent_fixed[ent < n_free_ent ? ent : 0] != 0 && !(CO && (ent == a.root_c || ent == a.root_m))); };
    double *set = a.ws + (size_t)a.parity * a.set_len, *other = a.ws + (size_t)(1 - a.parity) * a.set_len;
    const int nprev_raw = a.iters[0];
    {
        const int nprev = min(nprev_raw + 2, SPCG_BUFS);
        for (int bq = lane >> 3; bq < nprev; bq += 8) sp_st(other + (size_t)bq * a.stride + 8 * e + (lane & 7), __longlong_as_double((long long)SPCG_EMPTY));
    }
    if (fixed(e)) {
        if (lane < 6) sp_st(a.x_out + 6 * e + lane, 0.0);
        leave();
        return;
    }
    if (e == a.test_drop) return;
    int e0 = -1, n_act = 0;
#pragma unroll
    for (int k = 0; k < NEB; k++) {
        const unsigned long long fr = __ballot(lane + 64 * k < NENT && !fixed(lane + 64 * k));
        if (e0 < 0 && fr) e0 = 64 * k + __builtin_ctzll(fr);
        n_act += __builtin_popcountll(fr);
    }
    const double xcc = (double)(__builtin_amdgcn_s_getreg(20 | (0 << 6) | (3 << 11)) & 0xf);
    bool same_xcd = false;
    unsigned pact = 0;
#pragma unroll
    for (int k = 0; k < NL; k++) if (!fixed((lane + 64 * k) >> 2)) pact |= 1u << k;
    const bool ra = i < 6;
    const int row = 6 * e + (ra ? i : 0);
    double A2[2 * NK];
    double blk[6][6];
    double r, mi[6], zo[6];
    const bool pseudo = CO && (e == a.root_c || e == a.root_m);
    const int my_root = e < a.C ? a.root_c : (e < a.C + a.M ? a.root_m : -1);
    if (CO) {
        const double *rp = pseudo ? a.pre_azt + (size_t)((e == a.root_c ? 0 : 6) + (ra ? i : 0)) * a.n_pad : a.pre_rows + (size_t)row * a.n_pad;
#pragma unroll
        for (int k = 0; k < NK; k++) {
            const double2 t = reinterpret_cast<const double2 *>(rp)[8 * k + g];
            A2[2 * k] = ra ? t.x : 0.0; A2[2 * k + 1] = ra ? t.y : 0.0;
        }
#pragma unroll
        for (int k = 0; k < 3; k++) {
            const double2 t = reinterpret_cast<const double2 *>(a.pre_minv + 36 * e + 6 * (ra ? i : 0))[k];
            mi[2 * k] = (ra && !pseudo) ? t.x : 0.0; mi[2 * k + 1] = (ra && !pseudo) ? t.y : 0.0;
            const double2 z2 = reinterpret_cast<const double2 *>(a.pre_z + 36 * e + 6 * (ra ? i : 0))[k];
            const bool zon = ra && !pseudo && my_root >= 0;
            zo[2 * k] = zon ? z2.x : 0.0; zo[2 * k + 1] = zon ? z2.y : 0.0;
        }
        r = (ra && !pseudo) ? a.rhs[row] + a.g0[row] : 0.0;
    } else {
        unsigned long long cfx[(NK + 63) / 64] = {};
#pragma unroll
        for (int k = 0; k < NK; k++) {
            const int c0 = 16 * k + 2 * g, c1 = c0 + 1;
            A2[2 * k] = a.S[(c0 <= row) ? (size_t)row * a.n_pad + c0 : (size_t)c0 * a.n_pad + row];
            A2[2 * k + 1] = a.S[(c1 <= row) ? (size_t)row * a.n_pad + c1 : (size_t)c1 * a.n_pad + row];
            if (fixed(c0 / 6)) cfx[k >> 6] |= 1ull << (k & 63);
        }
#pragma unroll
        for (int p = 0; p < 6; p++)
#pragma unroll
            for (int q = 0; q <= p; q++) blk[p][q] = a.S[(size_t)(6 * e + p) * a.n_pad + 6 * e + q];
        r = a.rhs[row] + a.g0[row];
#pragma unroll
        for (int k = 0; k < NK; k++) {
            const int c0 = 16 * k + 2 * g;
            const bool off = !ra || ((cfx[k >> 6] >> (k & 63)) & 1);
            A2[2 * k] = off ? 0.0 : A2[2 * k] + (c0 == row ? a.mu : 0.0);
            A2[2 * k + 1] = off ? 0.0 : A2[2 * k + 1] + (c0 + 1 == row ? a.mu : 0.0);
        }
        if (!ra) r = 0.0;
    }
    SP_STAMP(0);
    SP_STAMP(1);
    if (!CO) {
        double inv[36];
#pragma unroll
        for (int p = 0; p < 6; p++) {
            blk[p][p] += a.mu;
#pragma unroll
            for (int q = 0; q < p; q++) blk[q][p] = blk[p][q];
        }
        if (!spd6_inverse(blk, inv) && lane == 0) atomicOr(a.flags, 2);
#pragma unroll
        for (int k = 0; k < 6; k++) {
            double v = 0.0;
#pragma unroll
            for (int p = 0; p < 6; p++) v = (i == p) ? inv[p * 6 + k] : v;
            mi[k] = v;
        }
    }
    double ec[12];
#pragma unroll
    for (int q = 0; q < 12; q++) ec[q] = 0.0;
    if (CO && pseudo) {
        const int Gq = e == a.root_c ? 0 : 1, elo = Gq ? a.C : 0, ehi = Gq ? a.C + a.M : a.C;
        const int ecl = lane & 7, sg = lane >> 3;
        double acc[10];
#pragma unroll
        for (int t = 0; t < 10; t++) acc[t] = 0.0;
        for (int q0 = elo; q0 < ehi; q0 += 40) {
            double2 v[5][5];
#pragma unroll
            for (int kk = 0; kk < 5; kk++) {
                const int q = q0 + 8 * kk + ecl;
#pragma unroll
                for (int t = 0; t < 5; t++) v[kk][t] = q < ehi ? reinterpret_cast<const double2 *>(a.pre_share + 80 * q + 10 * sg)[t] : make_double2(0.0, 0.0);
            }
#pragma unroll
            for (int kk = 0; kk < 5; kk++)
#pragma unroll
                for (int t = 0; t < 5; t++) { acc[2 * t] += v[kk][t].x; acc[2 * t + 1] += v[kk][t].y; }
        }
#pragma unroll
        for (int t = 0; t < 10; t++) acc[t] = sum8(acc[t]);
        if (ecl == 0) {
#pragma unroll
            for (int t = 0; t < 5; t++) reinterpret_cast<double2 *>(mv + 10 * sg)[t] = make_double2(acc[2 * t], acc[2 * t + 1]);
        }
        __builtin_amdgcn_wave_barrier();
        double eb[6][6], inv[36];
#pragma unroll
        for (int p = 0; p < 6; p++)
#pragma unroll
            for (int q = 0; q <= p; q++) { const double v = mv[12 * p + 6 * Gq + q]; eb[p][q] = v; eb[q][p] = v; }
        if (!spd6_inverse(eb, inv) && lane == 0) atomicOr(a.flags, 2);
#pragma unroll
        for (int k = 0; k < 6; k++) {
            double v = 0.0;
#pragma unroll
            for (int p = 0; p < 6; p++) v = (i == p) ? inv[p * 6 + k] : v;
            mi[k] = v;
        }
#pragma unroll
        for (int b = 0; b < 12; b++) ec[b] = ra ? mv[12 * i + b] : 0.0;
        r = ra ? mv[72 + i] : 0.0;
        __builtin_amdgcn_wave_barrier();
    }
    auto prec = [&](double w) -> double {
        double s = 0.0;
#pragma unroll
        for (int k = 0; k < 6; k++) s = fma(mi[k], rl(w, 8 * k), s);
        return s;
    };
    bool dead = false;
    auto publish = [&](int b, double val, double s1, double s2) {
        double *rec = set + (size_t)b * a.stride + 8 * e;
        double sh = (g & 1) ? s1 : s2;
        sh += dpp<DPP_ROR8>(sh);
        sh = sum_across_rows(sh);
        const bool is_m = ra && g == 0, is_s = lane == 1 || lane == 2;
        if (is_m || is_s) {
            if (same_xcd) sp_st_xcd(rec + (is_m ? i : 5 + lane), is_m ? val : sh);
            else sp_st(rec + (is_m ? i : 5 + lane), is_m ? val : sh);
        }
    };
    const __amdgpu_buffer_rsrc_t rsrc = __builtin_amdgcn_make_buffer_rsrc(set, 0, (int)(a.set_len * 8), 0x00020000);
    auto gather = [&](int b, double &t1, double &t2) {
        const int soff = b * a.stride * 8;
        double2 cur[NL];
#pragma unroll
        for (int k = 0; k < NL; k++) cur[k] = ((pact >> k) & 1) ? make_double2(__longlong_as_double((long long)SPCG_EMPTY), __longlong_as_double((long long)SPCG_EMPTY)) : make_double2(0.0, 0.0);
        long spins = 0;
        if (SPCG_PRE > 0) __builtin_amdgcn_s_sleep(SPCG_PRE);
        for (;;) {
            sp_u32x4 t[NL];
#pragma unroll
            for (int k = 0; k < NL; k++)
                if (sp_empty(cur[k].x) || sp_empty(cur[k].y)) t[k] = __builtin_amdgcn_raw_buffer_load_b128(rsrc, 16 * (lane + 64 * k), soff, 16 );
            bool ok = true;
#pragma unroll
            for (int k = 0; k < NL; k++) {
                if (sp_empty(cur[k].x) || sp_empty(cur[k].y)) {
                    const double lo = __hiloint2double((int)t[k][1], (int)t[k][0]), hi = __hiloint2double((int)t[k][3], (int)t[k][2]);
                    if (sp_empty(cur[k].x)) cur[k].x = lo;
                    if (sp_empty(cur[k].y)) cur[k].y = hi;
                    ok = ok && !sp_empty(cur[k].x) && !sp_empty(cur[k].y);
                }
            }
            if (__ballot(!ok) == 0ull) break;
#ifdef AAR_STAMPS
            if (e == e0 && lane == 0 && b < 80) g_sp_polls[b]++;
#endif
            if (++spins > (1L << 19)) { dead = true; break; }
            __builtin_amdgcn_s_sleep(1);
        }
        SP_STAMP(300 + b);
        const int w2 = lane & 3;
        double sg = 0.0, sd = 0.0;
#pragma unroll
        for (int k = 0; k < NL; k++) {
            if (w2 < 3) *reinterpret_cast<double2 *>(mv + 6 * ((lane + 64 * k) >> 2) + 2 * w2) = cur[k];
            else { sg += cur[k].x; sd += cur[k].y; }
        }
        const double sd_dn = dpp<0xF4>(sd);
        double sh = w2 == 3 ? sg : (w2 == 2 ? sd_dn : 0.0);
        sh += dpp<DPP_ROR4>(sh);
        sh += dpp<DPP_ROR8>(sh);
        sh = sum_across_rows(sh);
        t1 = rl(sh, 3); t2 = rl(sh, 2);
        __builtin_amdgcn_wave_barrier();
    };
    auto matvec = [&]() -> double {
        double s0 = 0.0, s1 = 0.0;
#pragma unroll
        for (int k = 0; k < NK; k++) {
            const double2 t = reinterpret_cast<const double2 *>(mv)[8 * k + g];
            s0 = fma(A2[2 * k], t.x, s0);
            s1 = fma(A2[2 * k + 1], t.y, s1);
        }
        if (CO && pseudo && g == 0) {
#pragma unroll
            for (int b = 0; b < 6; b++) {
                s0 = fma(ec[b], a.root_c >= 0 ? mv[6 * max(a.root_c, 0) + b] : 0.0, s0);
                s1 = fma(ec[6 + b], a.root_m >= 0 ? mv[6 * max(a.root_m, 0) + b] : 0.0, s1);
            }
        }
        const double s = sum8(s0 + s1);
        __builtin_amdgcn_wave_barrier();
        return s;
    };

    double x = 0.0;
    double u = prec(r), w = 0.0, z = 0.0, q = 0.0, s = 0.0, p = 0.0;
    double bb, d1;
    SP_STAMP(2);
    publish(0, u, r * u, i == 0 ? xcc + 4096.0 * xcc * xcc : 0.0);
    SP_STAMP(3);
    gather(0, bb, d1);
    SP_STAMP(4);
    {
        const double s2 = floor(d1 * (1.0 / 4096.0)), s1 = d1 - 4096.0 * s2;
        same_xcd = a.spread > 1 && (double)n_act * s2 == s1 * s1;
    }
    SP_VAL(400, bb); SP_VAL(401, d1); SP_VAL(402, u); SP_VAL(403, r); SP_VAL(404, mv[0]); SP_VAL(405, mv[6]); SP_VAL(406, mv[7]);
    int it = 0, status = 0;
    double uc = 0.0, qc = 0.0, pc = 0.0, xc = 0.0;
    const int rslot = (CO && my_root >= 0 && ra) ? 6 * my_root + i : 0;
    const bool track = CO && my_root >= 0 && ra && !pseudo;
    if (track) uc = mv[rslot];
    if (!dead) {
        w = matvec();
        SP_STAMP(6);
        double inv_g = 0.0, inv_a = 0.0;
        if (!(bb > 0.0)) status = 1;
        while (!status) {
            const double m = prec(w);
            SP_STAMP(8 + 4 * it);
            publish(it + 1, m, r * u, w * u);
            SP_STAMP(9 + 4 * it);
            double gam, dlt;
            gather(it + 1, gam, dlt);
            SP_STAMP(10 + 4 * it);
            if (it == 0) { SP_VAL(410, gam); SP_VAL(411, dlt); SP_VAL(412, m); SP_VAL(413, w); }
            if (dead) break;
            if (gam <= a.eta2 * bb && gam <= a.abs2_mu) { status = 1; break; }
            if (it >= a.max_it) { status = 2; break; }
            const double mc = track ? mv[rslot] : 0.0;
            const double nn = matvec();
            SP_STAMP(11 + 4 * it);
            const double beta = gam * inv_g;
            const double den = dlt - beta * gam * inv_a;
            if (!(den > 0.0) || !(gam > 0.0)) {
                status = (gam <= 1e-16 * bb) ? 1 : 3;
                break;
            }
            const double inv_den = rcp_refined(den);
            const double alpha = gam * inv_den;
            inv_a = den * (inv_g = rcp_refined(gam));
            z = fma(beta, z, nn);
            q = fma(beta, q, m);
            s = fma(beta, s, w);
            p = fma(beta, p, u);
            x = fma(alpha, p, x);
            r = fma(-alpha, s, r);
            u = fma(-alpha, q, u);
            w = fma(-alpha, z, w);
            if (CO) { qc = fma(beta, qc, mc); pc = fma(beta, pc, uc); xc = fma(alpha, pc, xc); uc = fma(-alpha, qc, uc); }
            it++;
        }
    }
    SP_STAMP(5);
    if (CO) {
#pragma unroll
        for (int q = 0; q < 6; q++) x = fma(zo[q], rl(xc, 8 * q), x);
        if (pseudo) x = 0.0;
    }
    if (ra && g == 0) sp_st(a.x_out + row, x);
    leave();
    if (lane == 0) {
        if (dead) atomicOr(a.flags, 4);
        if (status == 2 || status == 3) atomicOr(a.flags, 8);
        if (e == e0) {
            a.iters[0] = dead ? SPCG_BUFS : it;
            a.iters[1] += it;
            a.iters[2] += 1;
            if (status >= 2) a.iters[3] += 1;
            if (same_xcd) a.iters[4] += 1;
        }
    }
}

struct SpcgPreArgs {
    const double *S, *rhs, *g0;
    const double *ent;
    const int32_t *ent_fixed;
    int n, n_pad, n_ent, C, M, root_c, root_m;
    double mu;
    double *rows, *minv, *z;
    double *azt;
    double *share;
    int32_t *flags;
};

__device__ __forceinline__ void coarse_block(const double *__restrict__ row, bool on, double *__restrict__ Z) {
    const double *t = row + 9, *J = row + 12;
    const double c00 = J[4] * J[8] - J[5] * J[7], c01 = J[5] * J[6] - J[3] * J[8], c02 = J[3] * J[7] - J[4] * J[6];
    const double det = J[0] * c00 + J[1] * c01 + J[2] * c02;
    const double id = on ? 1.0 / det : 0.0, o1 = on ? 1.0 : 0.0;
#pragma unroll
    for (int q = 0; q < 36; q++) Z[q] = 0.0;
    Z[0] = c00 * id; Z[1] = (J[2] * J[7] - J[1] * J[8]) * id; Z[2] = (J[1] * J[5] - J[2] * J[4]) * id;
    Z[6] = c01 * id; Z[7] = (J[0] * J[8] - J[2] * J[6]) * id; Z[8] = (J[2] * J[3] - J[0] * J[5]) * id;
    Z[12] = c02 * id; Z[13] = (J[1] * J[6] - J[0] * J[7]) * id; Z[14] = (J[0] * J[4] - J[1] * J[3]) * id;
    Z[19] = o1 * t[2]; Z[20] = -o1 * t[1];
    Z[24] = -o1 * t[2]; Z[26] = o1 * t[0];
    Z[30] = o1 * t[1]; Z[31] = -o1 * t[0];
    Z[21] = o1; Z[28] = o1; Z[35] = o1;
}

__global__ void __launch_bounds__(256) k_spcg_pre(const SpcgPreArgs a) {
    extern __shared__ __align__(16) double sh[];
    const int tid = threadIdx.x, j = blockIdx.x;
    const int n_free_ent = a.n / 6, npose = a.C + a.M;
    if (j >= n_free_ent || a.ent_fixed[j]) return;
    double *zl = sh;
    double *al = zl + 36 * a.n_ent;
    double *az = al + 6 * a.n_pad;
    double *bj = az + 216;
    int32_t *fx = reinterpret_cast<int32_t *>(bj + 8);
    for (int q = tid; q < a.n_ent; q += 256) fx[q] = (q >= n_free_ent || a.ent_fixed[q < n_free_ent ? q : 0] != 0) ? 1 : 0;
    double er[12];
    {
        const bool pose = tid < npose && tid < a.n_ent;
#pragma unroll
        for (int q = 0; q < 12; q++) er[q] = pose ? a.ent[(size_t)tid * ENT_STRIDE + 9 + q] : 0.0;
    }
    {
        const int total = 6 * a.n_pad;
#pragma unroll 1
        for (int q0 = tid; q0 < total; q0 += 8 * 256) {
            double v[8];
#pragma unroll
            for (int k = 0; k < 8; k++) {
                const int q = q0 + 256 * k;
                if (q < total) {
                    const int i = q / a.n_pad, col = q - i * a.n_pad, row = 6 * j + i;
                    v[k] = a.S[(col <= row) ? (size_t)row * a.n_pad + col : (size_t)col * a.n_pad + row];
                }
            }
#pragma unroll
            for (int k = 0; k < 8; k++) {
                const int q = q0 + 256 * k;
                if (q < total) {
                    const int i = q / a.n_pad, col = q - i * a.n_pad, row = 6 * j + i;
                    al[q] = v[k] + (col == row ? a.mu : 0.0);
                }
            }
        }
    }
    for (int q = tid; q < a.n_ent; q += 256) {
        double Z[36], row[21];
        const bool pose = q < npose;
#pragma unroll
        for (int k = 0; k < 12; k++) row[9 + k] = q == tid ? er[k] : (pose ? a.ent[(size_t)q * ENT_STRIDE + 9 + k] : 0.0);
        coarse_block(row, pose && !(q >= n_free_ent || a.ent_fixed[q < n_free_ent ? q : 0] != 0), Z);
#pragma unroll
        for (int k = 0; k < 18; k++) reinterpret_cast<double2 *>(zl + 36 * q)[k] = make_double2(Z[2 * k], Z[2 * k + 1]);
    }
    if (tid < 6) bj[tid] = a.rhs[6 * j + tid] + a.g0[6 * j + tid];
    __syncthreads();
    for (int q = tid; q < 6 * a.n_pad; q += 256) { const int col = q % a.n_pad; if (fx[col / 6]) al[q] = 0.0; }
    __syncthreads();
    const bool pose = j < npose;
    if (tid >= 224) {
        if (tid == 224) {
            double blk[6][6], inv[36];
#pragma unroll
            for (int p = 0; p < 6; p++)
#pragma unroll
                for (int q = 0; q < 6; q++) blk[p][q] = al[p * a.n_pad + 6 * j + q];
            if (!spd6_inverse(blk, inv)) atomicOr(a.flags, 2);
#pragma unroll
            for (int q = 0; q < 36; q++) a.minv[36 * j + q] = inv[q];
        }
    } else if (tid < 216) {
        const int o = tid % 72, part = tid / 72, i = o / 12, c = o % 12;
        const int elo = c < 6 ? 0 : a.C, ehi = c < 6 ? a.C : npose, per = (ehi - elo + 2) / 3;
        const int lo = 6 * min(elo + part * per, ehi), hi = 6 * min(elo + (part + 1) * per, ehi);
        double acc = 0.0;
#pragma unroll 6
        for (int col = lo; col < hi; col++) acc = fma(al[i * a.n_pad + col], zl[6 * col + (c % 6)], acc);
        az[72 * part + o] = acc;
    }
    __syncthreads();
    if (tid < 72) {
        const int i = tid / 12, c = tid % 12;
        const double v = (az[tid] + az[72 + tid]) + az[144 + tid];
        az[tid] = v;
        a.azt[(size_t)c * a.n_pad + 6 * j + i] = v;
        const int root = c < 6 ? a.root_c : a.root_m;
        if (root >= 0) al[i * a.n_pad + 6 * root + (c % 6)] = v;
    }
    __syncthreads();
    for (int q = tid; q < 3 * a.n_pad; q += 256) reinterpret_cast<double2 *>(a.rows + (size_t)6 * j * a.n_pad)[q] = reinterpret_cast<const double2 *>(al)[q];
    const double *Zj = zl + 36 * j;
    if (tid < 36) a.z[36 * j + tid] = Zj[tid];
    if (pose && tid >= 64 && tid < 64 + 78) {
        const int o = tid - 64;
        double v = 0.0;
        if (o < 72) {
            const int c = o / 12, b = o % 12;
#pragma unroll
            for (int i = 0; i < 6; i++) v = fma(Zj[6 * i + c], az[12 * i + b], v);
        } else {
#pragma unroll
            for (int i = 0; i < 6; i++) v = fma(Zj[6 * i + (o - 72)], bj[i], v);
        }
        a.share[80 * j + o] = v;
    }
}

size_t spcg_pre_lds_bytes(int n_pad) { return sizeof(double) * ((size_t)36 * (n_pad / 6) + (size_t)6 * n_pad + 224) + sizeof(int32_t) * (n_pad / 6 + 2); }
size_t spcg_pre_doubles(int n_pad) { const size_t ne = n_pad / 6; return (size_t)n_pad * n_pad + 36 * ne + 36 * ne + (size_t)12 * n_pad + 80 * ne + 8; }

static void launch_spcg_pre(const DeviceProblem &P, int which, double mu, hipStream_t st, SpcgArgs &k) {
    const size_t ne = P.n_pad / 6;
    SpcgPreArgs a;
    a.S = P.blk[which].S; a.rhs = P.blk[which].rhs; a.g0 = P.blk[which].g0; a.ent = P.ent[which]; a.ent_fixed = P.ent_fixed;
    a.n = P.n; a.n_pad = P.n_pad; a.n_ent = (int)ne; a.C = P.C; a.M = P.M; a.mu = mu;
    a.root_c = P.spcg_root_c; a.root_m = P.spcg_root_m;
    double *w = P.spcg_pre;
    a.rows = w; w += (size_t)P.n_pad * P.n_pad;
    a.minv = w; w += 36 * ne;
    a.z = w; w += 36 * ne;
    a.azt = w; w += (size_t)12 * P.n_pad;
    a.share = w; w += 80 * ne;
    a.flags = P.flags;
    k.pre_rows = a.rows; k.pre_minv = a.minv; k.pre_z = a.z; k.pre_azt = a.azt; k.pre_share = a.share; k.root_c = a.root_c; k.root_m = a.root_m;
    HookScope _h(P, KID_SPCG_PRE);
    launch_lds(k_spcg_pre, dim3((unsigned)ne), dim3(256), spcg_pre_lds_bytes(P.n_pad), st, a);
}

bool spcg_fits(int nT) { return nT >= 1 && nT <= SPCG_MAX_NT; }
int spcg_resident_per_cu(int nT, bool coarse) {
    int nb = 0;
    hipError_t rc = hipErrorInvalidValue;
    switch (nT) {
#define SPCG_CASE(t) case t: { int nc = 1 << 30; if (coarse) rc = hipOccupancyMaxActiveBlocksPerMultiprocessor(&nc, k_spcg<t, true>, 64, 0); \
                               if (!coarse || rc == hipSuccess) rc = hipOccupancyMaxActiveBlocksPerMultiprocessor(&nb, k_spcg<t, false>, 64, 0); nb = std::min(nb, nc); } break;
        SPCG_CASE(1) SPCG_CASE(2) SPCG_CASE(3) SPCG_CASE(4) SPCG_CASE(5) SPCG_CASE(6) SPCG_CASE(7) SPCG_CASE(8)
        SPCG_CASE(9) SPCG_CASE(10) SPCG_CASE(11) SPCG_CASE(12) SPCG_CASE(13) SPCG_CASE(14)
#undef SPCG_CASE
        default: break;
    }
    if (rc != hipSuccess) { (void)hipGetLastError(); return 0; }
    return nb;
}
size_t spcg_ws_doubles(int n_pad) { return (size_t)2 * SPCG_BUFS * spcg_stride(n_pad); }
void spcg_ws_reset(const DeviceProblem &P, hipStream_t st) {
    (void)hipMemsetD32Async(reinterpret_cast<hipDeviceptr_t>(P.spcg_ws), (int)0xFFF85EED, 2 * spcg_ws_doubles(P.n_pad), st);
    (void)hipMemsetAsync(P.spcg_done, 0, 2 * sizeof(int32_t), st);
    P.spcg_epoch = 0;
}

bool launch_spcg(const DeviceProblem &P, int which, double mu, hipStream_t st, int trial) {
    const DeviceProblem::Blocks &b = P.blk[which];
    SpcgArgs a;
    a.S = b.S; a.rhs = b.rhs; a.g0 = b.g0; a.ent_fixed = P.ent_fixed; a.n = P.n; a.n_pad = P.n_pad;
    a.mu = mu; a.eta2 = P.pcg_eta_now * P.pcg_eta_now; a.abs2_mu = P.pcg_abs_tol * P.pcg_abs_tol * mu; a.max_it = std::min(P.spcg_max_it, SPCG_MAX_IT);
    a.ws = P.spcg_ws; a.stride = spcg_stride(P.n_pad); a.set_len = (long long)SPCG_BUFS * a.stride; a.parity = P.spcg_parity;
    a.x_out = P.delta_s; a.iters = P.spcg_iters; a.flags = P.flags; a.test_drop = P.spcg_test_drop;
    a.pre_rows = a.pre_minv = a.pre_z = a.pre_azt = a.pre_share = nullptr; a.root_c = a.root_m = -1; a.C = P.C; a.M = P.M;
    const bool coarse = spcg_coarse_now(P) && P.spcg_coarse_on;
    if (coarse) launch_spcg_pre(P, which, mu, st, a);
    a.spread = P.spcg_spread;
    P.spcg_parity ^= 1;
    const int n_ent = P.n_pad / 6;
    a.n_ent_total = n_ent;
    a.ride = (trial >= 0 && P.tune.spcg_backsub_rides && a.spread >= 8 && !P.hook.pre && P.F > 0) ? 1 : 0;
    a.bs = backsub_args(P, which, trial >= 0 ? trial : which, 1);
    a.done = P.spcg_done; a.done_epoch = 0; a.n_riders = 0;
    int grid = n_ent * a.spread;
    if (a.ride) {
        a.done_epoch = ++P.spcg_epoch;
        const int base = n_ent * (a.spread - 1), want = std::min(a.bs.n_frame_blocks + 1, 4096);
        int extra = 0;
        if (base < want) extra = ((want - base) * 8 + 6) / 7;
        grid += extra;
        a.n_riders = base + extra - (extra + 7) / 8;
    }
    HookScope _h(P, KID_SPCG);
    switch (P.nT) {
#define SPCG_CASE(t) case t: if (coarse) hipLaunchKernelGGL((k_spcg<t, true>), dim3(grid), dim3(64), 0, st, a); \
                             else hipLaunchKernelGGL((k_spcg<t, false>), dim3(grid), dim3(64), 0, st, a); break;
        SPCG_CASE(1) SPCG_CASE(2) SPCG_CASE(3) SPCG_CASE(4) SPCG_CASE(5) SPCG_CASE(6) SPCG_CASE(7) SPCG_CASE(8)
        SPCG_CASE(9) SPCG_CASE(10) SPCG_CASE(11) SPCG_CASE(12) SPCG_CASE(13) SPCG_CASE(14)
#undef SPCG_CASE
        default: break;
    }
    return a.ride != 0;
}

}
```

Measured before the change: 13380.

## Add 256-thread workgroup SPCG kernel that assembles coarse preconditioner in-kernel

```diff
diff --git a/automatic-ar_amd/csrc/ba_capi.hip b/automatic-ar_amd/csrc/ba_capi.hip
--- a/automatic-ar_amd/csrc/ba_capi.hip
+++ b/automatic-ar_amd/csrc/ba_capi.hip
@@ -1236,7 +1236,7 @@
         auto env_int = [](const char *name, int &v) { if (const char *e = getenv(name)) v = atoi(e); };
         env_int("AAR_FUSED_PANEL", P.tune.fused_panel); env_int("AAR_BS_RIDES", P.tune.bs_rides); env_int("AAR_BACKSUB_RIDES", P.tune.backsub_rides);
         env_int("AAR_LDL_LOOKAHEAD", P.tune.lookahead); env_int("AAR_PASSA_VARIANT", P.tune.passA_variant); env_int("AAR_PACK_SYSTEM", P.tune.pack_system);
-        env_int("AAR_INIT_HEADSTART", P.tune.init_headstart); env_int("AAR_PASSB_LEAN", P.tune.passB_lean); env_int("AAR_PASSA_WRENCH", P.tune.passA_wrench); env_int("AAR_PASSB_WRENCH_MERGED", P.tune.passB_wrench_merged); env_int("AAR_SPCG_BACKSUB_RIDES", P.tune.spcg_backsub_rides); env_int("AAR_PASSAB_OCC2", P.tune.passAB_occ2);
+        env_int("AAR_INIT_HEADSTART", P.tune.init_headstart); env_int("AAR_PASSB_LEAN", P.tune.passB_lean); env_int("AAR_PASSA_WRENCH", P.tune.passA_wrench); env_int("AAR_PASSB_WRENCH_MERGED", P.tune.passB_wrench_merged); env_int("AAR_SPCG_BACKSUB_RIDES", P.tune.spcg_backsub_rides); env_int("AAR_SPCG_WG4", P.tune.spcg_wg4); env_int("AAR_PASSAB_OCC2", P.tune.passAB_occ2);
     }
     const size_t ldsA = P.tune.passA_wrench ? passA_wrench_lds_bytes(P.max_kf, L.oi)
                                             : std::max(passA_lds_bytes(P.max_kf, 256), passA_lds_bytes(P.max_kf, 64));
@@ -1257,7 +1257,7 @@
         if (const char *t = getenv("AAR_PCG_E_EVERY")) P.pcg_e_every = std::max(1, atoi(t));
         if (const char *t = getenv("AAR_PCG_RESIDENT")) P.pcg_resident = atoi(t) != 0;
         if (pcg_lds_bytes(A, true) > 150 * 1024) P.pcg_coarse = 0;
-        const int spcg_per_cu = spcg_fits(P.nT) ? spcg_resident_per_cu(P.nT, spcg_coarse_now(P)) : 0;
+        const int spcg_per_cu = spcg_fits(P.nT) ? spcg_resident_per_cu(P.nT, spcg_coarse_now(P), P.tune.spcg_wg4 != 0) : 0;
         const bool spcg_ok = spcg_fits(P.nT) && P.n_pad / 6 <= std::max(1, spcg_per_cu) * cus;
         int solver = so.solver;
         if (solver == AAR_SOLVER_AUTO) {
@@ -1593,7 +1593,7 @@
     }
     if (P.use_spcg) {
         AL(spcg_ws, spcg_ws_doubles(P.n_pad)); AL(spcg_iters, 8); AL(spcg_done, 2);
-        if (spcg_coarse_now(P)) AL(spcg_pre, spcg_pre_doubles(P.n_pad));
+        if (spcg_coarse_now(P) && !P.tune.spcg_wg4) AL(spcg_pre, spcg_pre_doubles(P.n_pad));
         spcg_ws_reset(P, pb->stream);
     }
     if (P.n_smwork) { AL(Wd, (size_t)F * P.Ad * 36); AL(Yd, (size_t)F * P.Ad * 36); }
diff --git a/automatic-ar_amd/csrc/kernels.h b/automatic-ar_amd/csrc/kernels.h
--- a/automatic-ar_amd/csrc/kernels.h
+++ b/automatic-ar_amd/csrc/kernels.h
@@ -101,7 +101,6 @@
     int spcg_coarse_from = 12;
     mutable int spcg_coarse_on = 0;
     double *spcg_pre = nullptr;
-    mutable int spcg_pre_epoch = 0;
     int spcg_root_c = -1, spcg_root_m = -1, spcg_n_free = 0;
     int spcg_test_drop = -1;
     double *spcg_ws = nullptr;
@@ -118,6 +117,7 @@
         int passA_variant = 0;
         int passAB_occ2 = -1;
         int spcg_backsub_rides = 0;
+        int spcg_wg4 = 1;
         int passA_wrench = 1;
         int passB_wrench_merged = 0;
         int passB_lean = 0;
@@ -197,7 +197,7 @@
 size_t pcg_lds_bytes(int A, bool coarse = false);
 int pcg_max_grid(int A, bool coarse, int cus);
 bool launch_spcg(const DeviceProblem &P, int which, double mu, hipStream_t st, int trial = -1);
-int spcg_resident_per_cu(int nT, bool coarse);
+int spcg_resident_per_cu(int nT, bool coarse, bool wg4);
 inline bool spcg_coarse_now(const DeviceProblem &P) { return P.spcg_coarse && (P.spcg_root_c >= 0 || P.spcg_root_m >= 0); }
 bool spcg_fits(int nT);
 size_t spcg_ws_doubles(int n_pad);
diff --git a/automatic-ar_amd/csrc/spcg_kernels.hip b/automatic-ar_amd/csrc/spcg_kernels.hip
--- a/automatic-ar_amd/csrc/spcg_kernels.hip
+++ b/automatic-ar_amd/csrc/spcg_kernels.hip
@@ -8,6 +8,7 @@
 namespace {
 
 constexpr unsigned long long SPCG_EMPTY = 0xFFF85EEDFFF85EEDull;
+constexpr int SPCG_SHARE_REC = 152;
 
 __device__ __forceinline__ bool sp_empty(double v) { return (unsigned long long)__double_as_longlong(v) == SPCG_EMPTY; }
 __device__ __forceinline__ void sp_st(double *p, double v) { __hip_atomic_store(p, v, __ATOMIC_RELAXED, __HIP_MEMORY_SCOPE_AGENT); }
@@ -23,8 +24,8 @@
 #ifdef AAR_STAMPS
 __device__ unsigned long long g_sp_stamps[512];
 __device__ int g_sp_polls[80];
-#define SP_STAMP(k) do { __builtin_amdgcn_sched_barrier(0); if (e == e0 && lane == 0 && (k) < 512) g_sp_stamps[k] = __builtin_amdgcn_s_memtime(); __builtin_amdgcn_sched_barrier(0); } while (0)
-#define SP_VAL(k, v) do { if (e == e0 && lane == 0 && (k) < 512) g_sp_stamps[k] = (unsigned long long)__double_as_longlong(v); } while (0)
+#define SP_STAMP(k) do { __builtin_amdgcn_sched_barrier(0); if (e == e0 && tid == 0 && (k) < 512) g_sp_stamps[k] = __builtin_amdgcn_s_memtime(); __builtin_amdgcn_sched_barrier(0); } while (0)
+#define SP_VAL(k, v) do { if (e == e0 && tid == 0 && (k) < 512) g_sp_stamps[k] = (unsigned long long)__double_as_longlong(v); } while (0)
 #else
 #define SP_STAMP(k) do { } while (0)
 #define SP_VAL(k, v) do { } while (0)
@@ -32,6 +33,7 @@
 
 struct SpcgArgs {
     const double *S, *rhs, *g0;
+    const double *ent;
     const int32_t *ent_fixed;
     int n, n_pad;
     double mu, eta2;
@@ -40,6 +42,8 @@
     double *ws;
     long long set_len;
     int stride, parity;
+    double *shares;
+    long long share_len;
     double *x_out;
     int32_t *iters;
     int32_t *flags;
@@ -53,24 +57,171 @@
     int root_c, root_m;
     int C, M;
 };
-
 typedef unsigned int sp_u32x4 __attribute__((ext_vector_type(4)));
 
-template <int NT, bool CO>
-__global__ void __launch_bounds__(64) k_spcg(const SpcgArgs a) {
+struct SpcgPreArgs {
+    const double *S, *rhs, *g0;
+    const double *ent;
+    const int32_t *ent_fixed;
+    int n, n_pad, n_ent, C, M, root_c, root_m;
+    double mu;
+    double *rows, *minv, *z;
+    double *azt;
+    double *share;
+    int32_t *flags;
+};
+
+__device__ __forceinline__ void coarse_block(const double *__restrict__ row, bool on, double *__restrict__ Z) {
+    const double *t = row + 9, *J = row + 12;
+    const double c00 = J[4] * J[8] - J[5] * J[7], c01 = J[5] * J[6] - J[3] * J[8], c02 = J[3] * J[7] - J[4] * J[6];
+    const double det = J[0] * c00 + J[1] * c01 + J[2] * c02;
+    const double id = on ? 1.0 / det : 0.0, o1 = on ? 1.0 : 0.0;
+#pragma unroll
+    for (int q = 0; q < 36; q++) Z[q] = 0.0;
+    Z[0] = c00 * id; Z[1] = (J[2] * J[7] - J[1] * J[8]) * id; Z[2] = (J[1] * J[5] - J[2] * J[4]) * id;
+    Z[6] = c01 * id; Z[7] = (J[0] * J[8] - J[2] * J[6]) * id; Z[8] = (J[2] * J[3] - J[0] * J[5]) * id;
+    Z[12] = c02 * id; Z[13] = (J[1] * J[6] - J[0] * J[7]) * id; Z[14] = (J[0] * J[4] - J[1] * J[3]) * id;
+    Z[19] = o1 * t[2]; Z[20] = -o1 * t[1];
+    Z[24] = -o1 * t[2]; Z[26] = o1 * t[0];
+    Z[30] = o1 * t[1]; Z[31] = -o1 * t[0];
+    Z[21] = o1; Z[28] = o1; Z[35] = o1;
+}
+
+struct SpcgLds { double *zl, *al, *az, *bj, *minv; int32_t *fx; };
+__device__ __forceinline__ SpcgLds spcg_lds(double *sh, int n_ent, int n_pad, bool coarse) {
+    SpcgLds L;
+    L.zl = sh; L.al = sh + (coarse ? 36 * n_ent : 0); L.az = L.al + 6 * n_pad; L.bj = L.az + 216; L.minv = L.bj + 8;
+    L.fx = reinterpret_cast<int32_t *>(L.minv + 36);
+    return L;
+}
+size_t spcg_asm_lds_bytes(int n_pad, bool coarse) { return sizeof(double) * ((coarse ? (size_t)36 * (n_pad / 6) : 0) + (size_t)6 * n_pad + 260) + sizeof(int32_t) * (n_pad / 6 + 2); }
+
+template <bool COARSE>
+__device__ __forceinline__ void spcg_assemble(const SpcgPreArgs &a, int j, const SpcgLds &L) {
+    const int tid = threadIdx.x;
+    const int n_free_ent = a.n / 6, npose = a.C + a.M;
+    double *zl = L.zl, *al = L.al, *az = L.az, *bj = L.bj;
+    int32_t *fx = L.fx;
+    for (int q = tid; q < a.n_ent; q += 256) fx[q] = (q >= n_free_ent || a.ent_fixed[q < n_free_ent ? q : 0] != 0) ? 1 : 0;
+    double er[12];
+    if (COARSE) {
+        const bool pose = tid < npose && tid < a.n_ent;
+#pragma unroll
+        for (int q = 0; q < 12; q++) er[q] = pose ? a.ent[(size_t)tid * ENT_STRIDE + 9 + q] : 0.0;
+    }
+    {
+        const int total = 6 * a.n_pad;
+#pragma unroll 1
+        for (int q0 = tid; q0 < total; q0 += 8 * 256) {
+            double v[8];
+#pragma unroll
+            for (int k = 0; k < 8; k++) {
+                const int q = q0 + 256 * k;
+                if (q < total) {
+                    const int i = q / a.n_pad, col = q - i * a.n_pad, row = 6 * j + i;
+                    v[k] = a.S[(col <= row) ? (size_t)row * a.n_pad + col : (size_t)col * a.n_pad + row];
+                }
+            }
+#pragma unroll
+            for (int k = 0; k < 8; k++) {
+                const int q = q0 + 256 * k;
+                if (q < total) {
+                    const int i = q / a.n_pad, col = q - i * a.n_pad, row = 6 * j + i;
+                    al[q] = v[k] + (col == row ? a.mu : 0.0);
+                }
+            }
+        }
+    }
+    if (COARSE) {
+        for (int q = tid; q < a.n_ent; q += 256) {
+            double Z[36], row[21];
+            const bool pose = q < npose;
+#pragma unroll
+            for (int k = 0; k < 12; k++) row[9 + k] = q == tid ? er[k] : (pose ? a.ent[(size_t)q * ENT_STRIDE + 9 + k] : 0.0);
+            coarse_block(row, pose && !(q >= n_free_ent || a.ent_fixed[q < n_free_ent ? q : 0] != 0), Z);
+#pragma unroll
+            for (int k = 0; k < 18; k++) reinterpret_cast<double2 *>(zl + 36 * q)[k] = make_double2(Z[2 * k], Z[2 * k + 1]);
+        }
+    }
+    if (tid < 6) bj[tid] = a.rhs[6 * j + tid] + a.g0[6 * j + tid];
+    __syncthreads();
+    for (int q = tid; q < 6 * a.n_pad; q += 256) { const int col = q % a.n_pad; if (fx[col / 6]) al[q] = 0.0; }
+    __syncthreads();
+    if (tid >= 224) {
+        if (tid == 224) {
+            double blk[6][6], inv[36];
+#pragma unroll
+            for (int p = 0; p < 6; p++)
+#pragma unroll
+                for (int q = 0; q < 6; q++) blk[p][q] = al[p * a.n_pad + 6 * j + q];
+            if (!spd6_inverse(blk, inv)) atomicOr(a.flags, 2);
+#pragma unroll
+            for (int q = 0; q < 36; q++) L.minv[q] = inv[q];
+        }
+    } else if (COARSE && tid < 216) {
+        const int o = tid % 72, part = tid / 72, i = o / 12, c = o % 12;
+        const int elo = c < 6 ? 0 : a.C, ehi = c < 6 ? a.C : npose, per = (ehi - elo + 2) / 3;
+        const int lo = 6 * min(elo + part * per, ehi), hi = 6 * min(elo + (part + 1) * per, ehi);
+        double acc = 0.0;
+#pragma unroll 6
+        for (int col = lo; col < hi; col++) acc = fma(al[i * a.n_pad + col], zl[6 * col + (c % 6)], acc);
+        az[72 * part + o] = acc;
+    }
+    __syncthreads();
+    if (COARSE && tid < 72) {
+        const int i = tid / 12, c = tid % 12;
+        const double v = (az[tid] + az[72 + tid]) + az[144 + tid];
+        az[tid] = v;
+        const int root = c < 6 ? a.root_c : a.root_m;
+        if (root >= 0) al[i * a.n_pad + 6 * root + (c % 6)] = v;
+    }
+    __syncthreads();
+}
+
+__device__ __forceinline__ double spcg_share_entry(const double *Zj, const double *az, const double *bj, int o) {
+    double v = 0.0;
+    if (o < 72) {
+        const int c = o / 12, b = o % 12;
+#pragma unroll
+        for (int i = 0; i < 6; i++) v = fma(Zj[6 * i + c], az[12 * i + b], v);
+    } else {
+#pragma unroll
+        for (int i = 0; i < 6; i++) v = fma(Zj[6 * i + (o - 72)], bj[i], v);
+    }
+    return v;
+}
+
+template <int R, class At>
+__device__ __forceinline__ bool sp_poll(double (&v)[R], At at) {
+    long spins = 0;
+    for (;;) {
+#pragma unroll
+        for (int k = 0; k < R; k++) if (sp_empty(v[k])) v[k] = sp_ld(at(k));
+        bool ok = true;
+#pragma unroll
+        for (int k = 0; k < R; k++) ok = ok && !sp_empty(v[k]);
+        if (ok) return true;
+        if (++spins > (1L << 19)) return false;
+        __builtin_amdgcn_s_sleep(1);
+    }
+}
+
+template <int NT, bool CO, int NW, bool WG>
+__device__ __forceinline__ void spcg_entity(const SpcgArgs &a, double *mv, double *xw, double *area) {
     constexpr int NPAD = 96 * NT, NK = 6 * NT, NENT = 16 * NT, NL = NT, NEB = (NENT + 63) / 64;
-    __shared__ __align__(16) double mv[NPAD];
+    constexpr int KQ = (NK + NW - 1) / NW, LQ = (NL + NW - 1) / NW;
+    constexpr int NTHR = WG ? 256 : 64;
     if (blockIdx.x % a.spread || (int)blockIdx.x >= a.n_ent_total * a.spread) {
         if (!a.ride || blockIdx.x % 8 == 0) return;
-        __shared__ double red[32];
         const int bx = (int)blockIdx.x, cg_range = a.n_ent_total * a.spread;
         const int rid = bx < cg_range ? bx - bx / a.spread - 1 : a.n_ent_total * (a.spread - 1) + (bx - cg_range) - (bx - cg_range + 7) / 8;
-        for (int blk = rid; blk <= a.bs.n_frame_blocks; blk += a.n_riders) backsub_body(a.bs, blk, red, a.done + 1, a.done_epoch, a.flags);
+        for (int blk = rid; blk <= a.bs.n_frame_blocks; blk += a.n_riders) backsub_body(a.bs, blk, mv, a.done + 1, a.done_epoch, a.flags);
         return;
     }
-    const int lane = threadIdx.x, e = blockIdx.x / a.spread, i = lane >> 3, g = lane & 7;
+    const int tid = threadIdx.x, lane = tid & 63, wv = WG ? __builtin_amdgcn_readfirstlane(tid >> 6) : 0;
+    const int e = blockIdx.x / a.spread, i = lane >> 3, g = lane & 7;
     auto leave = [&]() {
-        if (!a.ride) return;
+        if (!a.ride || wv != 0) return;
         asm volatile("s_waitcnt vmcnt(0)" ::: "memory");
         if (lane == 0) {
             const int old = __hip_atomic_fetch_add(a.done, 1, __ATOMIC_RELAXED, __HIP_MEMORY_SCOPE_AGENT);
@@ -83,14 +234,67 @@
     const int nprev_raw = a.iters[0];
     {
         const int nprev = min(nprev_raw + 2, SPCG_BUFS);
-        for (int bq = lane >> 3; bq < nprev; bq += 8) sp_st(other + (size_t)bq * a.stride + 8 * e + (lane & 7), __longlong_as_double((long long)SPCG_EMPTY));
+        for (int bq = tid >> 3; bq < nprev; bq += NTHR / 8) sp_st(other + (size_t)bq * a.stride + 8 * e + (lane & 7), __longlong_as_double((long long)SPCG_EMPTY));
+        if (WG) for (int q = tid; q < SPCG_SHARE_REC; q += NTHR) sp_st(a.shares + (size_t)(1 - a.parity) * a.share_len + (size_t)SPCG_SHARE_REC * e + q, __longlong_as_double((long long)SPCG_EMPTY));
     }
     if (fixed(e)) {
-        if (lane < 6) sp_st(a.x_out + 6 * e + lane, 0.0);
+        if (tid < 6) sp_st(a.x_out + 6 * e + tid, 0.0);
         leave();
         return;
     }
     if (e == a.test_drop) return;
+    const bool ra = i < 6;
+    const int row = 6 * e + (ra ? i : 0);
+    const bool pseudo = CO && (e == a.root_c || e == a.root_m);
+    const int my_root = e < a.C ? a.root_c : (e < a.C + a.M ? a.root_m : -1);
+    bool dead = false;
+    const SpcgLds L = spcg_lds(area, NENT, NPAD, CO);
+    if (WG) {
+        if (tid < 64) xw[tid] = 0.0;
+        const double *recs = a.shares + (size_t)a.parity * a.share_len;
+        if (!pseudo) {
+            SpcgPreArgs pa;
+            pa.S = a.S; pa.rhs = a.rhs; pa.g0 = a.g0; pa.ent = a.ent; pa.ent_fixed = a.ent_fixed;
+            pa.n = a.n; pa.n_pad = NPAD; pa.n_ent = NENT; pa.C = a.C; pa.M = a.M; pa.root_c = a.root_c; pa.root_m = a.root_m; pa.mu = a.mu; pa.flags = a.flags;
+            spcg_assemble<CO>(pa, e, L);
+            if (CO) {
+                double *rec = a.shares + (size_t)a.parity * a.share_len + (size_t)SPCG_SHARE_REC * e;
+                if (tid < 72) sp_st(rec + tid, L.az[tid]);
+                else if (tid >= 128 && tid < 128 + 78 && e < a.C + a.M) sp_st(rec + 72 + (tid - 128), spcg_share_entry(L.zl + 36 * e, L.az, L.bj, tid - 128));
+            }
+        } else {
+            const int Gq = e == a.root_c ? 0 : 1, elo = Gq ? a.C : 0, ehi = Gq ? a.C + a.M : a.C;
+            for (int q = tid; q < NENT; q += 256) L.fx[q] = (q >= n_free_ent || a.ent_fixed[q < n_free_ent ? q : 0] != 0) ? 1 : 0;
+            for (int q = tid; q < 6 * NPAD; q += 256) L.al[q] = 0.0;
+            __syncthreads();
+            bool bad = false;
+#pragma unroll 1
+            for (int q0 = tid; q0 < 36 * NENT; q0 += 8 * 256) {
+                double v[8];
+#pragma unroll
+                for (int k = 0; k < 8; k++) { const int q = q0 + 256 * k; v[k] = (q < 36 * NENT && !L.fx[min(q / 36, NENT - 1)]) ? __longlong_as_double((long long)SPCG_EMPTY) : 0.0; }
+                if (!sp_poll(v, [&](int k) { const int q = q0 + 256 * k, o = q % 36; return recs + (size_t)SPCG_SHARE_REC * (q / 36) + 12 * (o / 6) + 6 * Gq + o % 6; })) bad = true;
+#pragma unroll
+                for (int k = 0; k < 8; k++) { const int q = q0 + 256 * k, o = q % 36; if (q < 36 * NENT) L.al[(o % 6) * NPAD + 6 * (q / 36) + o / 6] = v[k]; }
+            }
+            if (tid < 78) {
+                double acc = 0.0;
+#pragma unroll 1
+                for (int q0 = elo; q0 < ehi; q0 += 40) {
+                    double v[40];
+#pragma unroll
+                    for (int k = 0; k < 40; k++) v[k] = (q0 + k < ehi && !L.fx[min(q0 + k, NENT - 1)]) ? __longlong_as_double((long long)SPCG_EMPTY) : 0.0;
+                    if (!sp_poll(v, [&](int k) { return recs + (size_t)SPCG_SHARE_REC * (q0 + k) + 72 + tid; })) bad = true;
+#pragma unroll
+                    for (int k = 0; k < 40; k++) acc += v[k];
+                }
+                mv[tid] = acc;
+            }
+            if (bad) xw[12] = 1.0;
+            __syncthreads();
+            dead = xw[12] != 0.0;
+        }
+    }
     int e0 = -1, n_act = 0;
 #pragma unroll
     for (int k = 0; k < NEB; k++) {
@@ -102,15 +306,27 @@
     bool same_xcd = false;
     unsigned pact = 0;
 #pragma unroll
-    for (int k = 0; k < NL; k++) if (!fixed((lane + 64 * k) >> 2)) pact |= 1u << k;
-    const bool ra = i < 6;
-    const int row = 6 * e + (ra ? i : 0);
-    double A2[2 * NK];
+    for (int k = 0; k < LQ; k++) if (wv + NW * k < NL && !fixed((lane + 64 * (wv + NW * k)) >> 2)) pact |= 1u << k;
+    double A2[2 * KQ];
     double blk[6][6];
     double r, mi[6], zo[6];
-    const bool pseudo = CO && (e == a.root_c || e == a.root_m);
-    const int my_root = e < a.C ? a.root_c : (e < a.C + a.M ? a.root_m : -1);
-    if (CO) {
+    if (WG) {
+        const double *rp = L.al + (size_t)(ra ? i : 0) * NPAD;
+#pragma unroll
+        for (int k = 0; k < KQ; k++) {
+            const int kk = wv + NW * k;
+            const bool on = ra && kk < NK;
+            const double2 t = reinterpret_cast<const double2 *>(rp)[8 * min(kk, NK - 1) + g];
+            A2[2 * k] = on ? t.x : 0.0; A2[2 * k + 1] = on ? t.y : 0.0;
+        }
+        const bool zon = CO && ra && !pseudo && my_root >= 0;
+#pragma unroll
+        for (int k = 0; k < 6; k++) {
+            mi[k] = (ra && !pseudo) ? L.minv[6 * (ra ? i : 0) + k] : 0.0;
+            zo[k] = zon ? L.zl[36 * e + 6 * (ra ? i : 0) + k] : 0.0;
+        }
+        r = (ra && !pseudo) ? L.bj[ra ? i : 0] : 0.0;
+    } else if (CO) {
         const double *rp = pseudo ? a.pre_azt + (size_t)((e == a.root_c ? 0 : 6) + (ra ? i : 0)) * a.n_pad : a.pre_rows + (size_t)row * a.n_pad;
 #pragma unroll
         for (int k = 0; k < NK; k++) {
@@ -151,7 +367,7 @@
     }
     SP_STAMP(0);
     SP_STAMP(1);
-    if (!CO) {
+    if (!CO && !WG) {
         double inv[36];
 #pragma unroll
         for (int p = 0; p < 6; p++) {
@@ -172,57 +388,61 @@
 #pragma unroll
     for (int q = 0; q < 12; q++) ec[q] = 0.0;
     if (CO && pseudo) {
-        const int Gq = e == a.root_c ? 0 : 1, elo = Gq ? a.C : 0, ehi = Gq ? a.C + a.M : a.C;
-        const int ecl = lane & 7, sg = lane >> 3;
-        double acc[10];
-#pragma unroll
-        for (int t = 0; t < 10; t++) acc[t] = 0.0;
-        for (int q0 = elo; q0 < ehi; q0 += 40) {
-            double2 v[5][5];
-#pragma unroll
-            for (int kk = 0; kk < 5; kk++) {
-                const int q = q0 + 8 * kk + ecl;
-#pragma unroll
-                for (int t = 0; t < 5; t++) v[kk][t] = q < ehi ? reinterpret_cast<const double2 *>(a.pre_share + 80 * q + 10 * sg)[t] : make_double2(0.0, 0.0);
-            }
-#pragma unroll
-            for (int kk = 0; kk < 5; kk++)
-#pragma unroll
-                for (int t = 0; t < 5; t++) { acc[2 * t] += v[kk][t].x; acc[2 * t + 1] += v[kk][t].y; }
-        }
-#pragma unroll
-        for (int t = 0; t < 10; t++) acc[t] = sum8(acc[t]);
-        if (ecl == 0) {
-#pragma unroll
-            for (int t = 0; t < 5; t++) reinterpret_cast<double2 *>(mv + 10 * sg)[t] = make_double2(acc[2 * t], acc[2 * t + 1]);
-        }
-        __builtin_amdgcn_wave_barrier();
+        const int Gq = e == a.root_c ? 0 : 1;
+        if (!WG) {
+            const int elo = Gq ? a.C : 0, ehi = Gq ? a.C + a.M : a.C;
+            const int ecl = lane & 7, sg = lane >> 3;
+            double acc[10];
+#pragma unroll
+            for (int t = 0; t < 10; t++) acc[t] = 0.0;
+            for (int q0 = elo; q0 < ehi; q0 += 40) {
+                double2 v[5][5];
+#pragma unroll
+                for (int kk = 0; kk < 5; kk++) {
+                    const int q = q0 + 8 * kk + ecl;
+#pragma unroll
+                    for (int t = 0; t < 5; t++) v[kk][t] = q < ehi ? reinterpret_cast<const double2 *>(a.pre_share + 80 * q + 10 * sg)[t] : make_double2(0.0, 0.0);
+                }
+#pragma unroll
+                for (int kk = 0; kk < 5; kk++)
+#pragma unroll
+                    for (int t = 0; t < 5; t++) { acc[2 * t] += v[kk][t].x; acc[2 * t + 1] += v[kk][t].y; }
+            }
+#pragma unroll
+            for (int t = 0; t < 10; t++) acc[t] = sum8(acc[t]);
+            if (ecl == 0) {
+#pragma unroll
+                for (int t = 0; t < 5; t++) reinterpret_cast<double2 *>(mv + 10 * sg)[t] = make_double2(acc[2 * t], acc[2 * t + 1]);
+            }
+            __builtin_amdgcn_wave_barrier();
+        }
         double eb[6][6], inv[36];
 #pragma unroll
         for (int p = 0; p < 6; p++)
 #pragma unroll
             for (int q = 0; q <= p; q++) { const double v = mv[12 * p + 6 * Gq + q]; eb[p][q] = v; eb[q][p] = v; }
-        if (!spd6_inverse(eb, inv) && lane == 0) atomicOr(a.flags, 2);
+        const bool e_ok = spd6_inverse(eb, inv);
 #pragma unroll
         for (int k = 0; k < 6; k++) {
             double v = 0.0;
 #pragma unroll
             for (int p = 0; p < 6; p++) v = (i == p) ? inv[p * 6 + k] : v;
-            mi[k] = v;
-        }
-#pragma unroll
-        for (int b = 0; b < 12; b++) ec[b] = ra ? mv[12 * i + b] : 0.0;
+            mi[k] = e_ok ? v : 0.0;
+        }
+#pragma unroll
+        for (int b = 0; b < 12; b++) ec[b] = (ra && e_ok) ? mv[12 * i + b] : 0.0;
         r = ra ? mv[72 + i] : 0.0;
-        __builtin_amdgcn_wave_barrier();
-    }
+        if (WG) __syncthreads(); else __builtin_amdgcn_wave_barrier();
+    }
+    if (WG && NW == 1 && wv != 0) return;
     auto prec = [&](double w) -> double {
         double s = 0.0;
 #pragma unroll
         for (int k = 0; k < 6; k++) s = fma(mi[k], rl(w, 8 * k), s);
         return s;
     };
-    bool dead = false;
     auto publish = [&](int b, double val, double s1, double s2) {
+        if (NW > 1 && wv != 0) return;
         double *rec = set + (size_t)b * a.stride + 8 * e;
         double sh = (g & 1) ? s1 : s2;
         sh += dpp<DPP_ROR8>(sh);
@@ -236,19 +456,19 @@
     const __amdgpu_buffer_rsrc_t rsrc = __builtin_amdgcn_make_buffer_rsrc(set, 0, (int)(a.set_len * 8), 0x00020000);
     auto gather = [&](int b, double &t1, double &t2) {
         const int soff = b * a.stride * 8;
-        double2 cur[NL];
-#pragma unroll
-        for (int k = 0; k < NL; k++) cur[k] = ((pact >> k) & 1) ? make_double2(__longlong_as_double((long long)SPCG_EMPTY), __longlong_as_double((long long)SPCG_EMPTY)) : make_double2(0.0, 0.0);
+        double2 cur[LQ];
+#pragma unroll
+        for (int k = 0; k < LQ; k++) cur[k] = ((pact >> k) & 1) ? make_double2(__longlong_as_double((long long)SPCG_EMPTY), __longlong_as_double((long long)SPCG_EMPTY)) : make_double2(0.0, 0.0);
         long spins = 0;
         if (SPCG_PRE > 0) __builtin_amdgcn_s_sleep(SPCG_PRE);
         for (;;) {
-            sp_u32x4 t[NL];
-#pragma unroll
-            for (int k = 0; k < NL; k++)
-                if (sp_empty(cur[k].x) || sp_empty(cur[k].y)) t[k] = __builtin_amdgcn_raw_buffer_load_b128(rsrc, 16 * (lane + 64 * k), soff, 16 );
+            sp_u32x4 t[LQ];
+#pragma unroll
+            for (int k = 0; k < LQ; k++)
+                if (sp_empty(cur[k].x) || sp_empty(cur[k].y)) t[k] = __builtin_amdgcn_raw_buffer_load_b128(rsrc, 16 * (lane + 64 * (wv + NW * k)), soff, 16 );
             bool ok = true;
 #pragma unroll
-            for (int k = 0; k < NL; k++) {
+            for (int k = 0; k < LQ; k++) {
                 if (sp_empty(cur[k].x) || sp_empty(cur[k].y)) {
                     const double lo = __hiloint2double((int)t[k][1], (int)t[k][0]), hi = __hiloint2double((int)t[k][3], (int)t[k][2]);
                     if (sp_empty(cur[k].x)) cur[k].x = lo;
@@ -258,7 +478,7 @@
             }
             if (__ballot(!ok) == 0ull) break;
 #ifdef AAR_STAMPS
-            if (e == e0 && lane == 0 && b < 80) g_sp_polls[b]++;
+            if (e == e0 && tid == 0 && b < 80) g_sp_polls[b]++;
 #endif
             if (++spins > (1L << 19)) { dead = true; break; }
             __builtin_amdgcn_s_sleep(1);
@@ -267,8 +487,9 @@
         const int w2 = lane & 3;
         double sg = 0.0, sd = 0.0;
 #pragma unroll
-        for (int k = 0; k < NL; k++) {
-            if (w2 < 3) *reinterpret_cast<double2 *>(mv + 6 * ((lane + 64 * k) >> 2) + 2 * w2) = cur[k];
+        for (int k = 0; k < LQ; k++) {
+            if (NW > 1 && wv + NW * k >= NL) continue;
+            if (w2 < 3) *reinterpret_cast<double2 *>(mv + 6 * ((lane + 64 * (wv + NW * k)) >> 2) + 2 * w2) = cur[k];
             else { sg += cur[k].x; sd += cur[k].y; }
         }
         const double sd_dn = dpp<0xF4>(sd);
@@ -277,35 +498,53 @@
         sh += dpp<DPP_ROR8>(sh);
         sh = sum_across_rows(sh);
         t1 = rl(sh, 3); t2 = rl(sh, 2);
-        __builtin_amdgcn_wave_barrier();
+        if (NW > 1) {
+            if (lane == 0) { xw[2 * wv] = t1; xw[2 * wv + 1] = t2; xw[8 + wv] = dead ? 1.0 : 0.0; }
+            __syncthreads();
+            t1 = xw[0]; t2 = xw[1];
+            double dd = xw[8];
+#pragma unroll
+            for (int w = 1; w < NW; w++) { t1 += xw[2 * w]; t2 += xw[2 * w + 1]; dd += xw[8 + w]; }
+            dead = dd != 0.0;
+        } else {
+            __builtin_amdgcn_wave_barrier();
+        }
     };
     auto matvec = [&]() -> double {
         double s0 = 0.0, s1 = 0.0;
 #pragma unroll
-        for (int k = 0; k < NK; k++) {
-            const double2 t = reinterpret_cast<const double2 *>(mv)[8 * k + g];
+        for (int k = 0; k < KQ; k++) {
+            const double2 t = reinterpret_cast<const double2 *>(mv)[8 * min(wv + NW * k, NK - 1) + g];
             s0 = fma(A2[2 * k], t.x, s0);
             s1 = fma(A2[2 * k + 1], t.y, s1);
         }
-        if (CO && pseudo && g == 0) {
+        if (CO && pseudo && g == 0 && wv == 0) {
 #pragma unroll
             for (int b = 0; b < 6; b++) {
                 s0 = fma(ec[b], a.root_c >= 0 ? mv[6 * max(a.root_c, 0) + b] : 0.0, s0);
                 s1 = fma(ec[6 + b], a.root_m >= 0 ? mv[6 * max(a.root_m, 0) + b] : 0.0, s1);
             }
         }
-        const double s = sum8(s0 + s1);
-        __builtin_amdgcn_wave_barrier();
+        double s = sum8(s0 + s1);
+        if (NW > 1) {
+            if (g == 0) xw[16 + 8 * wv + i] = s;
+            __syncthreads();
+            s = xw[16 + i];
+#pragma unroll
+            for (int w = 1; w < NW; w++) s += xw[16 + 8 * w + i];
+        } else {
+            __builtin_amdgcn_wave_barrier();
+        }
         return s;
     };
 
     double x = 0.0;
     double u = prec(r), w = 0.0, z = 0.0, q = 0.0, s = 0.0, p = 0.0;
-    double bb, d1;
+    double bb = 0.0, d1 = 0.0;
     SP_STAMP(2);
-    publish(0, u, r * u, i == 0 ? xcc + 4096.0 * xcc * xcc : 0.0);
+    if (!dead) publish(0, u, r * u, i == 0 ? xcc + 4096.0 * xcc * xcc : 0.0);
     SP_STAMP(3);
-    gather(0, bb, d1);
+    if (!dead) gather(0, bb, d1);
     SP_STAMP(4);
     {
         const double s2 = floor(d1 * (1.0 / 4096.0)), s1 = d1 - 4096.0 * s2;
@@ -316,8 +555,8 @@
     double uc = 0.0, qc = 0.0, pc = 0.0, xc = 0.0;
     const int rslot = (CO && my_root >= 0 && ra) ? 6 * my_root + i : 0;
     const bool track = CO && my_root >= 0 && ra && !pseudo;
-    if (track) uc = mv[rslot];
     if (!dead) {
+        if (track) uc = mv[rslot];
         w = matvec();
         SP_STAMP(6);
         double inv_g = 0.0, inv_a = 0.0;
@@ -359,6 +598,7 @@
         }
     }
     SP_STAMP(5);
+    if (NW > 1 && wv != 0) return;
     if (CO) {
 #pragma unroll
         for (int q = 0; q < 6; q++) x = fma(zo[q], rl(xc, 8 * q), x);
@@ -379,137 +619,38 @@
     }
 }
 
-struct SpcgPreArgs {
-    const double *S, *rhs, *g0;
-    const double *ent;
-    const int32_t *ent_fixed;
-    int n, n_pad, n_ent, C, M, root_c, root_m;
-    double mu;
-    double *rows, *minv, *z;
-    double *azt;
-    double *share;
-    int32_t *flags;
-};
-
-__device__ __forceinline__ void coarse_block(const double *__restrict__ row, bool on, double *__restrict__ Z) {
-    const double *t = row + 9, *J = row + 12;
-    const double c00 = J[4] * J[8] - J[5] * J[7], c01 = J[5] * J[6] - J[3] * J[8], c02 = J[3] * J[7] - J[4] * J[6];
-    const double det = J[0] * c00 + J[1] * c01 + J[2] * c02;
-    const double id = on ? 1.0 / det : 0.0, o1 = on ? 1.0 : 0.0;
-#pragma unroll
-    for (int q = 0; q < 36; q++) Z[q] = 0.0;
-    Z[0] = c00 * id; Z[1] = (J[2] * J[7] - J[1] * J[8]) * id; Z[2] = (J[1] * J[5] - J[2] * J[4]) * id;
-    Z[6] = c01 * id; Z[7] = (J[0] * J[8] - J[2] * J[6]) * id; Z[8] = (J[2] * J[3] - J[0] * J[5]) * id;
-    Z[12] = c02 * id; Z[13] = (J[1] * J[6] - J[0] * J[7]) * id; Z[14] = (J[0] * J[4] - J[1] * J[3]) * id;
-    Z[19] = o1 * t[2]; Z[20] = -o1 * t[1];
-    Z[24] = -o1 * t[2]; Z[26] = o1 * t[0];
-    Z[30] = o1 * t[1]; Z[31] = -o1 * t[0];
-    Z[21] = o1; Z[28] = o1; Z[35] = o1;
-}
+template <int NT, bool CO>
+__global__ void __launch_bounds__(64) k_spcg(const SpcgArgs a) {
+    __shared__ __align__(16) double mv[96 * NT];
+    spcg_entity<NT, CO, 1, false>(a, mv, nullptr, nullptr);
+}
+
+#ifndef SPCG_WG_WAVES
+#define SPCG_WG_WAVES 4
+#endif
+template <int NT, bool CO>
+__global__ void __launch_bounds__(256) k_spcg_wg(const SpcgArgs a) {
+    extern __shared__ __align__(16) double sp_dyn[];
+    spcg_entity<NT, CO, SPCG_WG_WAVES, true>(a, sp_dyn, sp_dyn + 96 * NT, sp_dyn + 96 * NT + 64);
+}
+size_t spcg_wg_lds_bytes(int n_pad, bool coarse) { return sizeof(double) * ((size_t)n_pad + 64) + spcg_asm_lds_bytes(n_pad, coarse); }
 
 __global__ void __launch_bounds__(256) k_spcg_pre(const SpcgPreArgs a) {
     extern __shared__ __align__(16) double sh[];
     const int tid = threadIdx.x, j = blockIdx.x;
     const int n_free_ent = a.n / 6, npose = a.C + a.M;
     if (j >= n_free_ent || a.ent_fixed[j]) return;
-    double *zl = sh;
-    double *al = zl + 36 * a.n_ent;
-    double *az = al + 6 * a.n_pad;
-    double *bj = az + 216;
-    int32_t *fx = reinterpret_cast<int32_t *>(bj + 8);
-    for (int q = tid; q < a.n_ent; q += 256) fx[q] = (q >= n_free_ent || a.ent_fixed[q < n_free_ent ? q : 0] != 0) ? 1 : 0;
-    double er[12];
-    {
-        const bool pose = tid < npose && tid < a.n_ent;
-#pragma unroll
-        for (int q = 0; q < 12; q++) er[q] = pose ? a.ent[(size_t)tid * ENT_STRIDE + 9 + q] : 0.0;
-    }
-    {
-        const int total = 6 * a.n_pad;
-#pragma unroll 1
-        for (int q0 = tid; q0 < total; q0 += 8 * 256) {
-            double v[8];
-#pragma unroll
-            for (int k = 0; k < 8; k++) {
-                const int q = q0 + 256 * k;
-                if (q < total) {
-                    const int i = q / a.n_pad, col = q - i * a.n_pad, row = 6 * j + i;
-                    v[k] = a.S[(col <= row) ? (size_t)row * a.n_pad + col : (size_t)col * a.n_pad + row];
-                }
-            }
-#pragma unroll
-            for (int k = 0; k < 8; k++) {
-                const int q = q0 + 256 * k;
-                if (q < total) {
-                    const int i = q / a.n_pad, col = q - i * a.n_pad, row = 6 * j + i;
-                    al[q] = v[k] + (col == row ? a.mu : 0.0);
-                }
-            }
-        }
-    }
-    for (int q = tid; q < a.n_ent; q += 256) {
-        double Z[36], row[21];
-        const bool pose = q < npose;
-#pragma unroll
-        for (int k = 0; k < 12; k++) row[9 + k] = q == tid ? er[k] : (pose ? a.ent[(size_t)q * ENT_STRIDE + 9 + k] : 0.0);
-        coarse_block(row, pose && !(q >= n_free_ent || a.ent_fixed[q < n_free_ent ? q : 0] != 0), Z);
-#pragma unroll
-        for (int k = 0; k < 18; k++) reinterpret_cast<double2 *>(zl + 36 * q)[k] = make_double2(Z[2 * k], Z[2 * k + 1]);
-    }
-    if (tid < 6) bj[tid] = a.rhs[6 * j + tid] + a.g0[6 * j + tid];
-    __syncthreads();
-    for (int q = tid; q < 6 * a.n_pad; q += 256) { const int col = q % a.n_pad; if (fx[col / 6]) al[q] = 0.0; }
-    __syncthreads();
-    const bool pose = j < npose;
-    if (tid >= 224) {
-        if (tid == 224) {
-            double blk[6][6], inv[36];
-#pragma unroll
-            for (int p = 0; p < 6; p++)
-#pragma unroll
-                for (int q = 0; q < 6; q++) blk[p][q] = al[p * a.n_pad + 6 * j + q];
-            if (!spd6_inverse(blk, inv)) atomicOr(a.flags, 2);
-#pragma unroll
-            for (int q = 0; q < 36; q++) a.minv[36 * j + q] = inv[q];
-        }
-    } else if (tid < 216) {
-        const int o = tid % 72, part = tid / 72, i = o / 12, c = o % 12;
-        const int elo = c < 6 ? 0 : a.C, ehi = c < 6 ? a.C : npose, per = (ehi - elo + 2) / 3;
-        const int lo = 6 * min(elo + part * per, ehi), hi = 6 * min(elo + (part + 1) * per, ehi);
-        double acc = 0.0;
-#pragma unroll 6
-        for (int col = lo; col < hi; col++) acc = fma(al[i * a.n_pad + col], zl[6 * col + (c % 6)], acc);
-        az[72 * part + o] = acc;
-    }
-    __syncthreads();
-    if (tid < 72) {
-        const int i = tid / 12, c = tid % 12;
-        const double v = (az[tid] + az[72 + tid]) + az[144 + tid];
-        az[tid] = v;
-        a.azt[(size_t)c * a.n_pad + 6 * j + i] = v;
-        const int root = c < 6 ? a.root_c : a.root_m;
-        if (root >= 0) al[i * a.n_pad + 6 * root + (c % 6)] = v;
-    }
-    __syncthreads();
-    for (int q = tid; q < 3 * a.n_pad; q += 256) reinterpret_cast<double2 *>(a.rows + (size_t)6 * j * a.n_pad)[q] = reinterpret_cast<const double2 *>(al)[q];
-    const double *Zj = zl + 36 * j;
+    const SpcgLds L = spcg_lds(sh, a.n_ent, a.n_pad, true);
+    spcg_assemble<true>(a, j, L);
+    if (tid < 72) a.azt[(size_t)(tid % 12) * a.n_pad + 6 * j + tid / 12] = L.az[tid];
+    else if (tid < 108) a.minv[36 * j + tid - 72] = L.minv[tid - 72];
+    for (int q = tid; q < 3 * a.n_pad; q += 256) reinterpret_cast<double2 *>(a.rows + (size_t)6 * j * a.n_pad)[q] = reinterpret_cast<const double2 *>(L.al)[q];
+    const double *Zj = L.zl + 36 * j;
     if (tid < 36) a.z[36 * j + tid] = Zj[tid];
-    if (pose && tid >= 64 && tid < 64 + 78) {
-        const int o = tid - 64;
-        double v = 0.0;
-        if (o < 72) {
-            const int c = o / 12, b = o % 12;
-#pragma unroll
-            for (int i = 0; i < 6; i++) v = fma(Zj[6 * i + c], az[12 * i + b], v);
-        } else {
-#pragma unroll
-            for (int i = 0; i < 6; i++) v = fma(Zj[6 * i + (o - 72)], bj[i], v);
-        }
-        a.share[80 * j + o] = v;
-    }
-}
-
-size_t spcg_pre_lds_bytes(int n_pad) { return sizeof(double) * ((size_t)36 * (n_pad / 6) + (size_t)6 * n_pad + 224) + sizeof(int32_t) * (n_pad / 6 + 2); }
+    if (j < npose && tid >= 128 && tid < 128 + 78) a.share[80 * j + tid - 128] = spcg_share_entry(Zj, L.az, L.bj, tid - 128);
+}
+
+size_t spcg_pre_lds_bytes(int n_pad) { return spcg_asm_lds_bytes(n_pad, true); }
 size_t spcg_pre_doubles(int n_pad) { const size_t ne = n_pad / 6; return (size_t)n_pad * n_pad + 36 * ne + 36 * ne + (size_t)12 * n_pad + 80 * ne + 8; }
 
 static void launch_spcg_pre(const DeviceProblem &P, int which, double mu, hipStream_t st, SpcgArgs &k) {
@@ -525,18 +666,26 @@
     a.azt = w; w += (size_t)12 * P.n_pad;
     a.share = w; w += 80 * ne;
     a.flags = P.flags;
-    k.pre_rows = a.rows; k.pre_minv = a.minv; k.pre_z = a.z; k.pre_azt = a.azt; k.pre_share = a.share; k.root_c = a.root_c; k.root_m = a.root_m;
+    k.pre_rows = a.rows; k.pre_minv = a.minv; k.pre_z = a.z; k.pre_azt = a.azt; k.pre_share = a.share;
     HookScope _h(P, KID_SPCG_PRE);
     launch_lds(k_spcg_pre, dim3((unsigned)ne), dim3(256), spcg_pre_lds_bytes(P.n_pad), st, a);
 }
 
 bool spcg_fits(int nT) { return nT >= 1 && nT <= SPCG_MAX_NT; }
-int spcg_resident_per_cu(int nT, bool coarse) {
+int spcg_resident_per_cu(int nT, bool coarse, bool wg4) {
     int nb = 0;
     hipError_t rc = hipErrorInvalidValue;
+    auto ask = [&](auto kernel, int threads, size_t lds, int &n) {
+        raise_dynamic_lds(reinterpret_cast<const void *>(kernel), lds);
+        return hipOccupancyMaxActiveBlocksPerMultiprocessor(&n, kernel, threads, lds);
+    };
     switch (nT) {
-#define SPCG_CASE(t) case t: { int nc = 1 << 30; if (coarse) rc = hipOccupancyMaxActiveBlocksPerMultiprocessor(&nc, k_spcg<t, true>, 64, 0); \
-                               if (!coarse || rc == hipSuccess) rc = hipOccupancyMaxActiveBlocksPerMultiprocessor(&nb, k_spcg<t, false>, 64, 0); nb = std::min(nb, nc); } break;
+#define SPCG_CASE(t) case t: { int nc = 1 << 30; \
+                               if (wg4) { if (coarse) rc = ask(k_spcg_wg<t, true>, 256, spcg_wg_lds_bytes(96 * t, true), nc); \
+                                          if (!coarse || rc == hipSuccess) rc = ask(k_spcg_wg<t, false>, 256, spcg_wg_lds_bytes(96 * t, false), nb); } \
+                               else { if (coarse) rc = ask(k_spcg<t, true>, 64, 0, nc); \
+                                      if (!coarse || rc == hipSuccess) rc = ask(k_spcg<t, false>, 64, 0, nb); } \
+                               nb = std::min(nb, nc); } break;
         SPCG_CASE(1) SPCG_CASE(2) SPCG_CASE(3) SPCG_CASE(4) SPCG_CASE(5) SPCG_CASE(6) SPCG_CASE(7) SPCG_CASE(8)
         SPCG_CASE(9) SPCG_CASE(10) SPCG_CASE(11) SPCG_CASE(12) SPCG_CASE(13) SPCG_CASE(14)
 #undef SPCG_CASE
@@ -545,7 +694,7 @@
     if (rc != hipSuccess) { (void)hipGetLastError(); return 0; }
     return nb;
 }
-size_t spcg_ws_doubles(int n_pad) { return (size_t)2 * SPCG_BUFS * spcg_stride(n_pad); }
+size_t spcg_ws_doubles(int n_pad) { return (size_t)2 * SPCG_BUFS * spcg_stride(n_pad) + (size_t)2 * SPCG_SHARE_REC * (n_pad / 6); }
 void spcg_ws_reset(const DeviceProblem &P, hipStream_t st) {
     (void)hipMemsetD32Async(reinterpret_cast<hipDeviceptr_t>(P.spcg_ws), (int)0xFFF85EED, 2 * spcg_ws_doubles(P.n_pad), st);
     (void)hipMemsetAsync(P.spcg_done, 0, 2 * sizeof(int32_t), st);
@@ -554,20 +703,23 @@
 
 bool launch_spcg(const DeviceProblem &P, int which, double mu, hipStream_t st, int trial) {
     const DeviceProblem::Blocks &b = P.blk[which];
+    const bool wg4 = P.tune.spcg_wg4 != 0;
     SpcgArgs a;
-    a.S = b.S; a.rhs = b.rhs; a.g0 = b.g0; a.ent_fixed = P.ent_fixed; a.n = P.n; a.n_pad = P.n_pad;
+    a.S = b.S; a.rhs = b.rhs; a.g0 = b.g0; a.ent = P.ent[which]; a.ent_fixed = P.ent_fixed; a.n = P.n; a.n_pad = P.n_pad;
     a.mu = mu; a.eta2 = P.pcg_eta_now * P.pcg_eta_now; a.abs2_mu = P.pcg_abs_tol * P.pcg_abs_tol * mu; a.max_it = std::min(P.spcg_max_it, SPCG_MAX_IT);
     a.ws = P.spcg_ws; a.stride = spcg_stride(P.n_pad); a.set_len = (long long)SPCG_BUFS * a.stride; a.parity = P.spcg_parity;
+    a.share_len = (long long)SPCG_SHARE_REC * (P.n_pad / 6); a.shares = P.spcg_ws + 2 * a.set_len;
     a.x_out = P.delta_s; a.iters = P.spcg_iters; a.flags = P.flags; a.test_drop = P.spcg_test_drop;
     a.pre_rows = a.pre_minv = a.pre_z = a.pre_azt = a.pre_share = nullptr; a.root_c = a.root_m = -1; a.C = P.C; a.M = P.M;
     const bool coarse = spcg_coarse_now(P) && P.spcg_coarse_on;
-    if (coarse) launch_spcg_pre(P, which, mu, st, a);
+    if (coarse) { a.root_c = P.spcg_root_c; a.root_m = P.spcg_root_m; }
+    if (coarse && !wg4) launch_spcg_pre(P, which, mu, st, a);
     a.spread = P.spcg_spread;
     P.spcg_parity ^= 1;
     const int n_ent = P.n_pad / 6;
     a.n_ent_total = n_ent;
     a.ride = (trial >= 0 && P.tune.spcg_backsub_rides && a.spread >= 8 && !P.hook.pre && P.F > 0) ? 1 : 0;
-    a.bs = backsub_args(P, which, trial >= 0 ? trial : which, 1);
+    a.bs = backsub_args(P, which, trial >= 0 ? trial : which, wg4 ? 4 : 1);
     a.done = P.spcg_done; a.done_epoch = 0; a.n_riders = 0;
     int grid = n_ent * a.spread;
     if (a.ride) {
@@ -580,7 +732,9 @@
     }
     HookScope _h(P, KID_SPCG);
     switch (P.nT) {
-#define SPCG_CASE(t) case t: if (coarse) hipLaunchKernelGGL((k_spcg<t, true>), dim3(grid), dim3(64), 0, st, a); \
+#define SPCG_CASE(t) case t: if (wg4) { if (coarse) launch_lds(k_spcg_wg<t, true>, dim3(grid), dim3(256), spcg_wg_lds_bytes(96 * t, true), st, a); \
+                                        else launch_lds(k_spcg_wg<t, false>, dim3(grid), dim3(256), spcg_wg_lds_bytes(96 * t, false), st, a); } \
+                             else if (coarse) hipLaunchKernelGGL((k_spcg<t, true>), dim3(grid), dim3(64), 0, st, a); \
                              else hipLaunchKernelGGL((k_spcg<t, false>), dim3(grid), dim3(64), 0, st, a); break;
         SPCG_CASE(1) SPCG_CASE(2) SPCG_CASE(3) SPCG_CASE(4) SPCG_CASE(5) SPCG_CASE(6) SPCG_CASE(7) SPCG_CASE(8)
         SPCG_CASE(9) SPCG_CASE(10) SPCG_CASE(11) SPCG_CASE(12) SPCG_CASE(13) SPCG_CASE(14)
```

After: 12860. 0.961x the previous value.
